# chhylp123/hifiasm

Measured on AMD Instinct MI355X. Metric: read-pair overlaps/sec (sum ol->length / (ha_pt_gen + all-reads h_ec_lchain pass)), higher is better.
Workload: dtype u64 hashing / int32 + f64 chain scores

## Files before the change

### hifiasm_amd/csrc/hao_capi.hip

```cpp
#include <algorithm>
#include <cmath>
#include <cstring>
#include "hao_ctx.hpp"
#include "hao_sketch.cuh"
#include "hao_select2.cuh"
#include "hao_host.hpp"
#include "hao_index.cuh"
#include "hao_query.cuh"
#include "hao_chain.cuh"
#include "hao_deliver.cuh"
#include "hao_comm.hpp"
#include "hao_gather.hpp"
#include "hao_pipeline.hpp"
#include "hao_tables.hpp"
#include "hao_batch.hpp"
#include "hao_files.hpp"

extern "C" {

void hao_opt_default(hao_opt_t *o)
{
	memset(o, 0, sizeof(*o));
	o->k = 51; o->w = 51; o->hpc = 1; o->sample_dist = 500; o->rewin = 1000; o->min_hist_cnt = 5;
	o->max_kmer_cnt = 2000; o->max_n_chain = 100; o->high_factor = 5.0; o->is_ont = 0; o->hg_size = -1;
}

int hao_create(int device, const hao_opt_t *opt, hao_ctx **out)
{
	*out = nullptr;
	int n = 0;
	if (hipGetDeviceCount(&n) != hipSuccess || n <= 0 || device >= n) return HAO_ENODEV;
	if (hipSetDevice(device) != hipSuccess) return HAO_ENODEV;
	if (!opt || opt->k <= 0 || opt->k > 63 || opt->w <= 0 || opt->w >= 256) return HAO_EINVAL;
	hao_ctx *c = new hao_ctx();
	c->device = device; c->opt = *opt; c->max_n_chain = opt->max_n_chain; c->sw.load();
	{ int ncu = 0; if (hipDeviceGetAttribute(&ncu, hipDeviceAttributeMultiprocessorCount, device) == hipSuccess && ncu > 0) c->n_cu = ncu; }
	{
		int lo_ = 0, hi_ = 0; (void)hipDeviceGetStreamPriorityRange(&lo_, &hi_);
		if (hipStreamCreateWithPriority(&c->stream, hipStreamDefault, lo_) != hipSuccess) { delete c; return HAO_ENODEV; }
	}
	if (hipHostMalloc((void**)&c->peek_h, HAO_PEEK_WORDS * 8, hipHostMallocMapped) != hipSuccess || hipHostGetDevicePointer((void**)&c->peek_d, c->peek_h, 0) != hipSuccess) { (void)hipStreamDestroy(c->stream); delete c; return HAO_ENOMEM; }
	memset(c->ft_hist, 0, sizeof(c->ft_hist)); memset(c->pt_hist, 0, sizeof(c->pt_hist));
	*out = c;
	return HAO_OK;
}

void hao_destroy(hao_ctx *c)
{
	if (!c) return;
	(void)hipSetDevice(c->device);
	(void)hipStreamSynchronize(c->stream);
	delete c->batch; c->batch = nullptr;
	if (c->comm) { if (c->comm->nccl) ncclCommDestroy(c->comm->nccl); delete c->comm; c->comm = nullptr; }
	const hipStream_t st = c->stream; unsigned long long *const peek_h = c->peek_h;
	delete c;
	(void)hipStreamDestroy(st);
	if (peek_h) (void)hipHostFree(peek_h);
}

const char *hao_last_error(const hao_ctx *c) { return c ? c->err.c_str() : "null ctx"; }

#define HAO_NOT_ON_VIEW(c, what) do { if ((c)->owner) { hao_set_err((c), what ": not on an attached batch context (hao_attach)"); return HAO_EINVAL; } } while (0)

int hao_attach(hao_ctx *o, hao_ctx **out)
{
	if (!o || !out) return HAO_EINVAL;
	*out = nullptr;
	if (o->owner) { hao_set_err(o, "hao_attach: attach to the owning engine, not to another view"); return HAO_EINVAL; }
	hao_ctx *c = nullptr;
	if (int rc = hao_create(o->device, &o->opt, &c)) return rc;
	c->owner = o; c->attached_gen = ~0ULL;
	*out = c;
	return HAO_OK;
}

int hao_set_reads(hao_ctx *c, const uint8_t *packed, const uint64_t *pk_off, const uint32_t *len, uint64_t n_reads,
				  const uint64_t *nsite_off, const uint32_t *nsite)
{
	if (!c || !packed || !pk_off || !len) return HAO_EINVAL;
	HAO_NOT_ON_VIEW(c, "hao_set_reads"); ++c->index_gen;
	hao_gather_drop(c);
	if (n_reads >= (1ULL << 28)) { hao_set_err(c, "more than 2^28 reads (htab.cpp:765)"); return HAO_EUNSUPP; }
	HIP_TRY(hipSetDevice(c->device));
	c->n_reads = n_reads; c->n_pk_bytes = pk_off[n_reads]; c->max_len = 0;
	c->h_len.assign(len, len + n_reads);
	c->n_bases = 0;
	for (uint64_t i = 0; i < n_reads; ++i) {
		if (len[i] >= (1u << 27)) { hao_set_err(c, "read longer than 2^27 (htab.h:13-18)"); return HAO_EUNSUPP; }
		c->n_bases += len[i];
	}
	HIP_TRY(c->d_packed.reserve(c->n_pk_bytes + 16)); HIP_TRY(c->d_pk_off.reserve(n_reads + 1)); HIP_TRY(c->d_len.reserve(n_reads + 1));
	HIP_TRY(hipMemcpyAsync(c->d_packed.p, packed, c->n_pk_bytes, hipMemcpyHostToDevice, c->stream));
	HIP_TRY(hipMemsetAsync(c->d_packed.p + c->n_pk_bytes, 0, 16, c->stream));
	HIP_TRY(hipMemcpyAsync(c->d_pk_off.p, pk_off, (n_reads + 1) * 8, hipMemcpyHostToDevice, c->stream));
	HIP_TRY(hipMemcpyAsync(c->d_len.p, len, n_reads * 4, hipMemcpyHostToDevice, c->stream));
	c->has_n = nsite_off && nsite && nsite_off[n_reads] > 0;
	c->h_nsite_off.clear();
	if (c->has_n) {
		c->h_nsite_off.assign(nsite_off, nsite_off + n_reads + 1);
		HIP_TRY(c->d_nsite_off.reserve(n_reads + 1)); HIP_TRY(c->d_nsite.reserve(nsite_off[n_reads] + 1));
		HIP_TRY(hipMemcpyAsync(c->d_nsite_off.p, nsite_off, (n_reads + 1) * 8, hipMemcpyHostToDevice, c->stream));
		HIP_TRY(hipMemcpyAsync(c->d_nsite.p, nsite, nsite_off[n_reads] * 4, hipMemcpyHostToDevice, c->stream));
	}
	c->rid_base = 0; c->n_total = n_reads; c->h_len_all = c->h_len;
	c->max_len_all = 0; for (uint64_t i = 0; i < n_reads; ++i) c->max_len_all = std::max(c->max_len_all, len[i]);
	HIP_TRY(c->d_len_all.reserve(n_reads + 1));
	HIP_TRY(hipMemcpyAsync(c->d_len_all.p, len, n_reads * 4, hipMemcpyHostToDevice, c->stream));
	HIP_TRY(hipStreamSynchronize(c->stream));
	c->has_ft = false; c->has_pt = false; c->h_ix_valid = false; c->sk_n = 0;
	return HAO_OK;
}

int hao_set_shard(hao_ctx *c, uint64_t rid_base, uint64_t n_total, const uint32_t *all_len)
{
	if (!c || !all_len || rid_base + c->n_reads > n_total) return HAO_EINVAL;
	HAO_NOT_ON_VIEW(c, "hao_set_shard"); ++c->index_gen;
	hao_gather_drop(c);
	if (n_total >= (1ULL << 28)) { hao_set_err(c, "more than 2^28 reads (htab.cpp:765)"); return HAO_EUNSUPP; }
	for (uint64_t i = 0; i < c->n_reads; ++i) if (all_len[rid_base + i] != c->h_len[i]) { hao_set_err(c, "all_len disagrees with the local read lengths"); return HAO_EINVAL; }
	HIP_TRY(hipSetDevice(c->device));
	c->rid_base = rid_base; c->n_total = n_total; c->h_len_all.assign(all_len, all_len + n_total); c->max_len = 0;
	c->max_len_all = 0; for (uint64_t i = 0; i < n_total; ++i) c->max_len_all = std::max(c->max_len_all, all_len[i]);
	HIP_TRY(c->d_len_all.reserve(n_total + 1));
	HIP_TRY(hipMemcpy(c->d_len_all.p, all_len, n_total * 4, hipMemcpyHostToDevice));
	c->has_ft = false; c->has_pt = false; c->h_ix_valid = false;
	return HAO_OK;
}

int hao_dist_unique_id(uint8_t id[128])
{
	ncclUniqueId u; if (ncclGetUniqueId(&u) != ncclSuccess) return HAO_ENODEV;
	static_assert(sizeof(ncclUniqueId) <= 128, "ncclUniqueId");
	memset(id, 0, 128); memcpy(id, &u, sizeof(u));
	return HAO_OK;
}

int hao_dist_init(hao_ctx *c, const uint8_t id[128], int rank, int world)
{
	if (!c || !id || rank < 0 || rank >= world) return HAO_EINVAL;
	HAO_NOT_ON_VIEW(c, "hao_dist_init");
	HIP_TRY(hipSetDevice(c->device));
	if (!c->comm) c->comm = new hao_comm();
	ncclUniqueId u; memcpy(&u, id, sizeof(u));
	c->comm->rank = rank; c->comm->world = world; c->comm->loop = nullptr;
	{
		int rt = 0; NCCL_TRY(ncclGetVersion(&rt));
		const int rt_major = rt >= 10000 ? rt / 10000 : rt / 1000;
		if (rt_major != NCCL_MAJOR) { hao_set_err(c, "RCCL major version " + std::to_string(rt_major) + " at run time, " + std::to_string(NCCL_MAJOR) + " at compile time"); return HAO_EUNSUPP; }
	}
	NCCL_TRY(ncclCommInitRank(&c->comm->nccl, world, u, rank));
	return HAO_OK;
}

void *hao_loop_create(int world)
{
	hao_loop_group *g = new hao_loop_group();
	g->world = world; pthread_barrier_init(&g->bar, nullptr, world); g->ptr.assign(world, nullptr); g->ptr2.assign(world, nullptr); g->cnt.resize(world); g->hostv.resize(world);
	return g;
}
void hao_loop_destroy(void *grp) { if (grp) { hao_loop_group *g = (hao_loop_group*)grp; pthread_barrier_destroy(&g->bar); delete g; } }
int hao_dist_init_loopback(hao_ctx *c, void *grp, int rank)
{
	if (!c || !grp) return HAO_EINVAL;
	hao_loop_group *g = (hao_loop_group*)grp;
	if (rank < 0 || rank >= g->world) return HAO_EINVAL;
	if (!c->comm) c->comm = new hao_comm();
	c->comm->rank = rank; c->comm->world = g->world; c->comm->loop = g; c->comm->nccl = nullptr;
	return HAO_OK;
}

int hao_sketch_batch(hao_ctx *c, uint64_t rid_lo, uint64_t rid_hi, int use_ft, int sample_dist)
{
	if (!c || rid_lo > rid_hi || rid_hi > c->n_reads) return HAO_EINVAL;
	HAO_NOT_ON_VIEW(c, "hao_sketch_batch");
	HIP_TRY(hipSetDevice(c->device));
	c->timer.begin(c->stream);
	int rc = hao_sketch_run(c, rid_lo, rid_hi, use_ft && c->has_ft, sample_dist, 1);
	if (rc != HAO_OK) return rc;
	HIP_TRY(hipStreamSynchronize(c->stream));
	c->timer.collect(c->stage_ms);
	c->h_mz_off.resize(c->sk_n + 1);
	HIP_TRY(hipMemcpy(c->h_mz_off.data(), c->d_mz_off.p, (c->sk_n + 1) * 8, hipMemcpyDeviceToHost));
	return HAO_OK;
}

int hao_fetch_sketch(hao_ctx *c, uint64_t rid, const hao_mz_t **mz, uint64_t *n)
{
	if (!c || rid < c->sk_lo || rid >= c->sk_lo + c->sk_n || c->h_mz_off.size() != c->sk_n + 1) return HAO_EINVAL;
	HIP_TRY(hipSetDevice(c->device));
	uint64_t s = c->h_mz_off[rid - c->sk_lo], e = c->h_mz_off[rid - c->sk_lo + 1], m = e - s;
	c->h_mz_fetch.resize(m + 1);
	std::vector<uint64_t> x(m + 1), info(m + 1);
	if (m) {
		HIP_TRY(hipMemcpy(x.data(), c->d_mz_x.p + s, m * 8, hipMemcpyDeviceToHost));
		HIP_TRY(hipMemcpy(info.data(), c->d_mz_info.p + s, m * 8, hipMemcpyDeviceToHost));
	}
	for (uint64_t i = 0; i < m; ++i) { c->h_mz_fetch[i].x = x[i]; c->h_mz_fetch[i].info = info[i]; }
	*mz = c->h_mz_fetch.data(); *n = m;
	return HAO_OK;
}

int hao_stage_times(hao_ctx *c, const char **names, float *ms, int cap)
{
	if (!c) return 0;
	int n = 0;
	for (auto &p : c->stage_ms) { if (n >= cap) break; names[n] = p.first.c_str(); ms[n] = p.second; ++n; }
	return n;
}

}

#include "hao_capi_rest.hpp"
#include "hao_sortdbg.hpp"
```

### hifiasm_amd/csrc/hao_ctx.hpp

```cpp
#pragma once
#include <time.h>
#include <rocprim/rocprim.hpp>
#include <map>
#include <algorithm>
#include <cstdlib>
#include <cstring>
#include <type_traits>
#include "hao_common.cuh"
#include "hao_grid_pair.cuh"

struct hao_ctx;
static void hao_set_err(hao_ctx *c, const std::string &m);

template<typename T> struct DevBuf {
	T *p = nullptr; size_t cap = 0; bool borrowed = false;
	DevBuf() = default;
	DevBuf(const DevBuf&) = delete; DevBuf &operator=(const DevBuf&) = delete;
	DevBuf(DevBuf &&o) noexcept : p(o.p), cap(o.cap), borrowed(o.borrowed) { o.p = nullptr; o.cap = 0; o.borrowed = false; }
	DevBuf &operator=(DevBuf &&o) noexcept { if (this != &o) { release(); p = o.p; cap = o.cap; borrowed = o.borrowed; o.p = nullptr; o.cap = 0; o.borrowed = false; } return *this; }
	~DevBuf() { release(); }
	hipError_t reserve(size_t n) {
		if (n <= cap) return hipSuccess;
		if (borrowed) return hipErrorInvalidValue;
		if (p) (void)hipFree(p);
		p = nullptr; cap = 0;
		size_t want = n + n / 8 + 64;
		hipError_t e = hipMalloc((void**)&p, want * sizeof(T));
		if (e == hipSuccess) cap = want;
		return e;
	}
	hipError_t reserve_exact(size_t n) {
		if (n <= cap) return hipSuccess;
		if (borrowed) return hipErrorInvalidValue;
		if (p) (void)hipFree(p);
		p = nullptr; cap = 0;
		hipError_t e = hipMalloc((void**)&p, n * sizeof(T));
		if (e == hipSuccess) cap = n;
		return e;
	}
	void release() { if (p && !borrowed) (void)hipFree(p); p = nullptr; cap = 0; borrowed = false; }
	void borrow(const DevBuf<T> &o) { release(); p = o.p; cap = o.cap; borrowed = o.p != nullptr; }
};

inline bool hao_dbg_sync = false;
struct StageTimer {
	std::vector<std::string> names; std::vector<hipEvent_t> ev; std::vector<double> host_t; hipStream_t st = nullptr;
	static double now() { struct timespec ts; clock_gettime(CLOCK_MONOTONIC, &ts); return ts.tv_sec + 1e-9 * ts.tv_nsec; }
	void begin(hipStream_t s) { st = s; names.clear(); host_t.clear(); mark("__begin"); }
	void mark(const char *name) {
		size_t i = names.size();
		if (i >= ev.size()) { hipEvent_t e; (void)hipEventCreate(&e); ev.push_back(e); }
		names.push_back(name); host_t.push_back(now()); (void)hipEventRecord(ev[i], st);
		if (hao_dbg_sync) { const hipError_t e = hipStreamSynchronize(st); fprintf(stderr, "[stage] %s: %s\n", name, hipGetErrorString(e)); fflush(stderr); }
	}
	void collect(std::vector<std::pair<std::string, float> > &out) {
		out.clear();
		for (size_t i = 1; i < names.size(); ++i) { float ms = 0; (void)hipEventElapsedTime(&ms, ev[i - 1], ev[i]); out.push_back(std::make_pair(names[i], ms)); }
		for (size_t i = 1; i < names.size(); ++i) if (names[i].compare(0, 3, "ft_") == 0) out.push_back(std::make_pair("host_" + names[i], (float)((host_t[i] - host_t[i - 1]) * 1e3)));
	}
	~StageTimer() { for (auto e : ev) (void)hipEventDestroy(e); }
};

struct hao_switches {
	bool seedphase = false, qcphase = false, dp_stats = false, selphase = false, dltime = false, bloom = false;
	bool seq_chain = false, dp_seqtail = false, dp_nospec = false, dp_serial = false, seq_prune = false, seed_noql = false, al_coop = false;
	long long sk_gcap = -1, exc_cap = -1, ft_chunk_slots = 0; unsigned long long gather_chunk = 64ULL << 20, al_slice = 4ULL << 30, ix_pad = 0, sort40_min = 1ULL << 23; int fc_raw_every = 0, exc_every = 0; bool qmz_raw = false, arena_probe = false;
	int arena_numa = 3, seed_merge_maxn = 24000, seed_lds_ratio = 120, ft_passes = 0, seed_lds = 1;
	static bool in_list(const char *v, const char *name) {
		const size_t n = strlen(name);
		for (const char *p = v; p && *p; ) { const char *e = strchr(p, ','); const size_t l = e ? (size_t)(e - p) : strlen(p); if (l == n && strncmp(p, name, n) == 0) return true; p = e ? e + 1 : nullptr; }
		return false;
	}
	static bool in_kv(const char *v, const char *name, unsigned long long &out) {
		const size_t n = strlen(name);
		for (const char *p = v; p && *p; ) { const char *e = strchr(p, ','); if (strncmp(p, name, n) == 0 && p[n] == '=') { out = strtoull(p + n + 1, nullptr, 10); return true; } p = e ? e + 1 : nullptr; }
		return false;
	}
	void load() {
		if (const char *v = getenv("HAO_DBG_PRINT")) {
			seedphase = in_list(v, "seed"); qcphase = in_list(v, "qc"); dp_stats = in_list(v, "dp"); selphase = in_list(v, "sel"); dltime = in_list(v, "dl"); bloom = in_list(v, "bloom"); hao_dbg_sync = in_list(v, "sync");
		}
		if (const char *v = getenv("HAO_DBG_FORCE")) {
			seq_chain = in_list(v, "seq_chain");
			dp_seqtail = in_list(v, "dp_seqtail");
			dp_nospec = in_list(v, "dp_nospec");
			dp_serial = in_list(v, "dp_serial");
			seq_prune = in_list(v, "seq_prune");
			seed_noql = in_list(v, "noql");
			al_coop = in_list(v, "al_coop");
		}
		if (const char *v = getenv("HAO_DBG_TEST")) {
			unsigned long long x;
			if (in_kv(v, "ix_pad", x)) ix_pad = x;
			if (in_kv(v, "sort40_min", x)) sort40_min = x;
			if (in_kv(v, "sk_gcap", x)) sk_gcap = (long long)x;
			if (in_kv(v, "exc_cap", x)) exc_cap = (long long)x;
			if (in_kv(v, "fc_raw_every", x)) fc_raw_every = (int)x;
			if (in_kv(v, "exc_every", x)) exc_every = (int)x;
			if (in_kv(v, "qmz_raw", x)) qmz_raw = x != 0;
			if (in_kv(v, "arena_probe", x)) arena_probe = x != 0;
			if (in_kv(v, "ft_chunk_slots", x)) ft_chunk_slots = (long long)x;
			if (in_kv(v, "al_slice", x)) al_slice = std::max<unsigned long long>(x, 8);
			if (in_kv(v, "gather_chunk", x)) gather_chunk = std::max<unsigned long long>(x, 64);
		}
		if (const char *e = getenv("HAO_SEED_LDS")) seed_lds = atoi(e) ? 1 : 0;
		if (const char *e = getenv("HAO_SEED_LDS_RATIO")) seed_lds_ratio = std::max(0, atoi(e));
		if (const char *e = getenv("HAO_SEED_MERGE_MAXN")) seed_merge_maxn = std::max(0, atoi(e));
		if (const char *e = getenv("HAO_FT_PASSES")) ft_passes = std::max(0, atoi(e));
		if (const char *e = getenv("HAO_ARENA_NUMA")) arena_numa = atoi(e);
	}
};

static __global__ void hao_peek_kernel(const unsigned long long *src, int n, unsigned long long *dst)
{ if ((int)threadIdx.x < n) dst[threadIdx.x] = src[threadIdx.x]; }
enum hao_peek_id : int {
	PK_ANCHORS, PK_CLS_BASE,
	PK_N_CHAINS, PK_N_CL, PK_N_FC_RAW, PK_N_OL, PK_N_FC,
	PK_N_EXC, PK_N_CODES, PK_N_FCW, PK_SEED_OVF, PK_ERR, PK_SLOW,
	PK_GRID_PAIRS, PK_REF_SLOTS, PK_REF_UNRES,
	PK_SORT40,
	PK_TG_TRACED, PK_TG_CTR, PK_TG_NCIG,
	PK_RS_SIZES, PK_RS_WAITING, PK_RS_TOTAL, PK_RS_NWINS,
	PK_WL_N, PK_WL_PLAN, PK_WL_NCIG, PK_WL_CTR,
	PK_LD_SETUP, PK_LD_ROUND, PK_LD_SEL, PK_LD_END,
	PK_COUNT
};
struct hao_peek_rng { int at, n; };
static constexpr hao_peek_rng HAO_PEEK[PK_COUNT] = {
	 {0, 1},  {1, 8},
	 {9, 1},  {10, 1},  {11, 1},  {12, 1},  {13, 1},
	 {14, 1},  {15, 1},  {19, 1},  {20, 3},  {23, 1},  {64, 11},
	 {32, 1},  {37, 1},  {38, 1},
	 {16, 3},
	 {33, 1},  {34, 2},  {36, 1},
	 {40, 2},  {42, 1},  {43, 1},  {44, 1},
	 {48, 1},  {49, 3},  {52, 1},  {53, 6},
	 {80, 2},  {82, 48},  {130, 16},  {146, 2},
};
constexpr int HAO_PEEK_WORDS = 512;
constexpr bool hao_peek_table_ok()
{
	for (int i = 0; i < PK_COUNT; ++i) {
		if (HAO_PEEK[i].at < 0 || HAO_PEEK[i].n < 1 || HAO_PEEK[i].at + HAO_PEEK[i].n > HAO_PEEK_WORDS) return false;
		for (int j = 0; j < i; ++j) if (HAO_PEEK[i].at < HAO_PEEK[j].at + HAO_PEEK[j].n && HAO_PEEK[j].at < HAO_PEEK[i].at + HAO_PEEK[i].n) return false;
	}
	return true;
}
static_assert(hao_peek_table_ok(), "read-back slots: a range beyond the mapped words, or two ranges that overlap");

struct WinResident {
	enum Stage { NONE, ED, RESCUE, WLIST };
	void on_new_batch() { *this = WinResident(); }
	void on_host_fed() { owner = NOBODY; n = 0; trace = false; }
	void on_grid(uint64_t pairs) { owner = GRID; n = pairs; lists = false; }
	void on_ref_begin(Stage s) { if (chain >= s) chain = (Stage)(s - 1); host &= (1u << s) - 1; if (s == ED) { owner = NOBODY; n = 0; } lists = false; }
	void on_ref_done(Stage s, uint64_t pairs = 0) { chain = s; if (s == ED) { owner = REF; n = pairs; } if (s == WLIST) lists = true; }
	void on_host_copy(Stage s) { host |= 1u << s; }
	void on_trace_grid(bool done) { trace = done; }
	uint64_t scratch_pairs() const { return owner == NOBODY ? 0 : n; }
	bool ed_resident() const { return chain >= ED; } bool rescue_resident() const { return chain >= RESCUE; } bool trace_resident() const { return trace; }
	bool ref_input_resident() const { return chain >= ED && owner == REF; }
	bool wlist_input_resident() const { return chain >= RESCUE && owner == REF; }
	bool wlist_resident() const { return chain >= WLIST && owner == REF; }
	bool wlist_records_resident() const { return lists; }
	bool host_current(Stage s) const { return (host >> s) & 1u; }
private:
	enum Owner { NOBODY, GRID, REF } owner = NOBODY; uint64_t n = 0; Stage chain = NONE; uint32_t host = 0; bool trace = false, lists = false;
};

struct hao_ref_io {
	const hao_ovlp_t *ol; uint64_t n_ol;
	uint32_t wl; const uint8_t *tab;
	const hao_ed_pair *pairs; uint64_t n_pairs, n_slots;
	const hao_ed_result_t *res; const uint8_t *err8; const uint16_t *pe16;
	DevBuf<hao_rs_ovlp> *rs_ovlp; DevBuf<uint64_t> *rs_off; DevBuf<hao_rs_win> *rs_wins;
	DevBuf<uint64_t> *wl_woff; DevBuf<hao_rs_win> *wl_wins; DevBuf<uint64_t> *wl_cigoff; DevBuf<uint16_t> *wl_cig;
};

struct hao_ctx {
	int device = 0; hao_opt_t opt; std::string err; hipStream_t stream = nullptr; hao_switches sw;
	hao_ctx *owner = nullptr; uint64_t index_gen = 0, attached_gen = 0;
	unsigned long long *peek_h = nullptr, *peek_d = nullptr;
	unsigned long long peeked(hao_peek_id slot, int k = 0) const { return peek_h[HAO_PEEK[slot].at + k]; }
	uint64_t n_reads = 0, n_bases = 0, n_pk_bytes = 0; bool has_n = false; uint32_t max_len = 0;
	DevBuf<uint8_t> d_packed; DevBuf<uint64_t> d_pk_off; DevBuf<uint32_t> d_len; DevBuf<uint64_t> d_nsite_off; DevBuf<uint32_t> d_nsite;
	std::vector<uint32_t> h_len; std::vector<uint64_t> h_nsite_off;
	uint64_t rid_base = 0, n_total = 0; uint32_t max_len_all = 0; int n_cu = 256; DevBuf<uint32_t> d_len_all; std::vector<uint32_t> h_len_all; struct hao_comm *comm = nullptr;
	bool gs_valid = false, gs_has_n = false; uint64_t gs_pk_bytes = 0, gs_nsites = 0;
	DevBuf<uint8_t> g_packed; DevBuf<uint64_t> g_pk_off, g_nsite_off; DevBuf<uint32_t> g_nsite;
	bool has_ft = false; int ft_peak_hom = -1, ft_peak_het = -1, ft_cutoff = 0, ft_passes_used = 1; int64_t ft_hist[HAO_N_COUNTS];
	std::vector<uint64_t> h_ft_keys; std::vector<int32_t> h_ft_vals;
	DevBuf<uint64_t> d_ft_keys; DevBuf<int32_t> d_ft_vals; DevBuf<uint32_t> d_ft_bucket;
	DevBuf<uint32_t> d_ft_hbit; DevBuf<unsigned long long> d_ft_hslot; int ft_hbits = 0;
	int max_n_chain = 100, hom_cov = -1, het_cov = -1;
	uint64_t sk_lo = 0, sk_n = 0, sk_total = 0; bool sk_is_index = false;
	DevBuf<uint64_t> d_tile_off; DevBuf<uint32_t> d_tile_ord, d_n_runs, d_tot_l; DevBuf<uint64_t> d_chunk_off, d_chunk_cnt64;
	DevBuf<uint8_t> d_scalar_flag; DevBuf<uint32_t> d_scalar_list, d_unit_rid;
	DevBuf<uint64_t> d_pool_x, d_pool_info; DevBuf<uint32_t> d_pool_ord; DevBuf<unsigned long long> d_cursor; DevBuf<int> d_err;
	DevBuf<uint64_t> d_chunk_base, d_chunk_dst; DevBuf<uint32_t> d_chunk_cnt;
	DevBuf<uint64_t> d_g_x, d_g_info; DevBuf<uint32_t> d_g_ord; DevBuf<uint64_t> d_g_off; DevBuf<uint32_t> d_new_n; DevBuf<uint64_t> d_new_n64;
	DevBuf<uint64_t> d_mz_x, d_mz_info, d_mz_off;
	DevBuf<unsigned char> d_tmp; DevBuf<unsigned char> d_ring; DevBuf<uint32_t> d_ringord, d_cnt_ws;
	std::vector<uint64_t> h_mz_off; std::vector<hao_mz_t> h_mz_fetch;
	bool has_pt = false; int64_t pt_hist[HAO_N_COUNTS];
	uint64_t ix_n_mz = 0, ix_n_sorted = 0, ix_n_keys = 0, ix_n_pos = 0, ix_pad = 0; int ix_bucket_bits = 16;
	DevBuf<uint64_t> d_ix_mz_x, d_ix_mz_info, d_ix_mz_off;
	DevBuf<uint64_t> d_ix_sx, d_ix_sinfo;
	DevBuf<uint64_t> d_ix_lk; bool lk_valid = false; DevBuf<uint32_t> w_runid;
	DevBuf<uint64_t> d_ix_keys, d_ix_start; DevBuf<uint32_t> d_ix_cnt; DevBuf<uint32_t> d_ix_bucket;
	DevBuf<uint64_t> w_ukeys, w_flag, w_kpos, w_ustart; DevBuf<uint32_t> w_ucnt; DevBuf<unsigned long long> w_hist; DevBuf<uint32_t> w_ok, w_ok2, w_oi, w_oi2;
	DevBuf<uint32_t> w_s40_list, w_s40_o; DevBuf<uint64_t> w_s40_x, w_lkv2; DevBuf<unsigned long long> w_s40_cnt; uint64_t s40_runs = 0;
	std::vector<uint64_t> h_ix_keys, h_ix_off, h_ix_pos, h_ix_mz_off; bool h_ix_valid = false;
	WinResident win;
	DevBuf<hao_ed_task_t> al_task; DevBuf<uint64_t> al_k1, al_k2, al_path; DevBuf<uint32_t> al_i1, al_order, al_sel; DevBuf<hao_ed_result_t> al_res; DevBuf<hao_trace_result_t> al_tres;
	DevBuf<uint8_t> al_want; DevBuf<uint16_t> al_cig;
	uint32_t ded_window = 0, ded_thre = 0;
	uint32_t ded_place = 0; double ded_erate = 0; DevBuf<uint8_t> ded_tab;
	struct RefGrid {
		DevBuf<uint64_t> cnt, woff; DevBuf<int16_t> shift; DevBuf<uint8_t> werr; DevBuf<hao_ed_pair> pairs; DevBuf<unsigned long long> ctr;
	} rf;
	DevBuf<uint8_t> rf_tab; uint32_t rf_tab_wl = 0; double rf_tab_erate = 0; DevBuf<hao_ed_ovlp_sum> rf_sum; std::vector<hao_ed_ovlp_sum> rf_hsum; uint64_t rf_unres = 0, rs_wc = 0;
	struct Rescue {
		DevBuf<uint16_t> wpe; DevBuf<uint64_t> rbase, path, off; DevBuf<hao_rs_state> st; DevBuf<hao_rs_win> rec, wins; DevBuf<hao_rs_ovlp> ovlp; DevBuf<unsigned long long> ctr;
		std::vector<hao_rs_ovlp> h_ovlp; std::vector<uint64_t> h_win_off; std::vector<hao_rs_win> h_wins;
	} rs;
	uint64_t rs_slots = 0, rs_rounds = 0, rs_active = 0, rs_total = 0, rs_nw = 0;
	struct Wlist {
		DevBuf<uint64_t> cnt, woff, ncig, cig_off, key, key2, path; DevBuf<hao_wl_plan> plan; DevBuf<hao_rs_win> wins; DevBuf<uint32_t> idx, sel, rowof; DevBuf<uint16_t> rows, cig; DevBuf<unsigned long long> ctr;
		std::vector<uint64_t> h_woff, h_cig_off, r_woff, r_cig_off; std::vector<hao_rs_win> h_wins; std::vector<uint16_t> h_cig;
	} wl;
	uint64_t wl_out[5] = { 0, 0, 0, 0, 0 };
	struct Ladder {
		DevBuf<hao_ladder_req_t> req; DevBuf<hao_ladder_res_t> res; DevBuf<int32_t> att; DevBuf<uint64_t> ncig, rowref, off, poff, selcnt; DevBuf<uint32_t> open[2], sel; DevBuf<hao_ld_coord> coord;
		DevBuf<uint16_t> rows[5], cig; DevBuf<unsigned long long> ctr;
		DevBuf<hao_ladder_adv_res_t> res_adv; DevBuf<uint32_t> xlist; DevBuf<uint16_t> xrow; DevBuf<int32_t> pth;
		DevBuf<int64_t> est;
		DevBuf<hao_ladder_req_t> e_req; DevBuf<int64_t> e_est; DevBuf<unsigned long long> e_ctr;
	} ld;
	uint64_t ld_n = 0;
	bool ld_valid = false, ld_adv = false; uint64_t ld_ncig = 0, ld_rounds[5] = { 0, 0, 0, 0, 0 };
	struct TraceGrid {
		DevBuf<uint8_t> want; DevBuf<uint32_t> sel; DevBuf<uint64_t> cnt, loc, off, path; DevBuf<uint16_t> rows; DevBuf<unsigned long long> ctr;
	} tg;
	uint32_t tg_wl = 0, tg_thre = 0; uint64_t tg_n = 0, tg_nsel = 0, tg_ncig = 0, tg_nuntr = 0;
	DevBuf<hao_ed_pair> tg_pairs; DevBuf<uint8_t> tg_err; DevBuf<uint16_t> tg_pe, tg_ps, tg_ncig16, tg_cig;
	struct Batch;
	Batch *batch = nullptr;
	StageTimer timer; std::vector<std::pair<std::string, float> > stage_ms;
};

static void hao_set_err(hao_ctx *c, const std::string &m) { if (c) c->err = m; }

#define HAO_CHECK_LAUNCH() HIP_TRY(hipGetLastError())

static int hao_peek(hao_ctx *c, const void *src, int words, hao_peek_id slot)
{
	if (words > HAO_PEEK[slot].n) { hao_set_err(c, "hao_peek: more words than the slot holds"); return HAO_EINVAL; }
	hipLaunchKernelGGL(hao_peek_kernel, dim3(1), dim3(64), 0, c->stream, (const unsigned long long*)src, words, c->peek_d + HAO_PEEK[slot].at); HAO_CHECK_LAUNCH();
	return HAO_OK;
}

static bool hao_comm_is_active(const struct hao_comm *cm);
static inline bool hao_is_sharded(const hao_ctx *c) { const hao_ctx *o = c->owner ? c->owner : c; return o->comm && hao_comm_is_active(o->comm); }

struct hao_read_view {
	const uint8_t *packed; const uint64_t *pk_off; const uint32_t *len; const uint64_t *nsite_off; const uint32_t *nsite;
	const uint32_t *h_len; uint64_t n, id_base, local0;
};
static inline bool hao_reads_view(const hao_ctx *c, hao_read_view *V)
{
	if (!hao_is_sharded(c)) {
		V->packed = c->d_packed.p; V->pk_off = c->d_pk_off.p; V->len = c->d_len.p; V->nsite_off = c->has_n ? c->d_nsite_off.p : nullptr; V->nsite = c->has_n ? c->d_nsite.p : nullptr;
		V->h_len = c->h_len.data(); V->n = c->n_reads; V->id_base = c->rid_base; V->local0 = 0;
		return true;
	}
	if (!c->gs_valid) return false;
	V->packed = c->g_packed.p; V->pk_off = c->g_pk_off.p; V->len = c->d_len_all.p; V->nsite_off = c->gs_has_n ? c->g_nsite_off.p : nullptr; V->nsite = c->gs_has_n ? c->g_nsite.p : nullptr;
	V->h_len = c->h_len_all.data(); V->n = c->n_total; V->id_base = 0; V->local0 = c->rid_base;
	return true;
}
#define HAO_STAGE_VIEW(c, V, what) hao_read_view V; do { if (!hao_reads_view((c), &V)) { hao_set_err((c), what ": single-device mode only"); return HAO_EUNSUPP; } } while (0)

static inline hipError_t hao_tmp(hao_ctx *c, size_t bytes) { return c->d_tmp.reserve(bytes + 256); }

template<typename F>
static int hao_rocprim(hao_ctx *c, F run)
{
	size_t tb = 0;
	HIP_TRY(run((void*)nullptr, tb));
	HIP_TRY(hao_tmp(c, tb));
	HIP_TRY(run((void*)c->d_tmp.p, tb));
	return HAO_OK;
}
template<typename In, typename Out>
static int hao_excl_scan_u64(hao_ctx *c, In in, Out out, size_t n)
{
	return hao_rocprim(c, [&](void *tmp, size_t &tb) { return rocprim::exclusive_scan(tmp, tb, in, out, (uint64_t)0, n, rocprim::plus<uint64_t>(), c->stream); });
}
template<typename K, typename V>
static int hao_sort_pairs(hao_ctx *c, K *k_in, K *k_out, V *v_in, V *v_out, size_t n, unsigned bits)
{
	return hao_rocprim(c, [&](void *tmp, size_t &tb) { return rocprim::radix_sort_pairs(tmp, tb, k_in, k_out, v_in, v_out, n, 0, bits, c->stream); });
}
template<typename In, typename F, typename Out>
static int hao_select(hao_ctx *c, In in, F flags_or_pred, Out out, uint64_t *count, size_t n)
{
	return hao_rocprim(c, [&](void *tmp, size_t &tb) {
		if constexpr (std::is_pointer<F>::value) return rocprim::select(tmp, tb, in, flags_or_pred, out, count, n, c->stream);
		else return rocprim::select(tmp, tb, in, out, count, n, flags_or_pred, c->stream);
	});
}

static inline uint64_t hao_col_slice(const hao_ctx *c, uint64_t n, uint64_t bytes_per_pair)
{
	return std::max<uint64_t>(256, std::min<uint64_t>((n + 255) & ~255ULL, (c->sw.al_slice / bytes_per_pair) & ~255ULL));
}
#define HAO_SCRATCH_KEEP (1ULL << 30)
template<typename T> static inline void hao_release_above(DevBuf<T> &b, uint64_t bytes) { if ((uint64_t)b.cap * sizeof(T) > bytes) b.release(); }

static int hao_view_refresh(hao_ctx *c)
{
	hao_ctx *o = c->owner;
	if (!o || c->attached_gen == o->index_gen) return HAO_OK;
	c->opt = o->opt;
	c->n_reads = o->n_reads; c->n_bases = o->n_bases; c->n_pk_bytes = o->n_pk_bytes; c->has_n = o->has_n; c->max_len = o->max_len;
	c->rid_base = o->rid_base; c->n_total = o->n_total; c->max_len_all = o->max_len_all; c->n_cu = o->n_cu; c->max_n_chain = o->max_n_chain; c->hom_cov = o->hom_cov; c->het_cov = o->het_cov;
	c->has_pt = o->has_pt; c->ix_n_mz = o->ix_n_mz; c->ix_n_sorted = o->ix_n_sorted; c->ix_n_keys = o->ix_n_keys; c->ix_n_pos = o->ix_n_pos; c->ix_pad = o->ix_pad; c->ix_bucket_bits = o->ix_bucket_bits; c->lk_valid = o->lk_valid;
	c->h_len = o->h_len; c->h_nsite_off = o->h_nsite_off; c->h_len_all = o->h_len_all; c->h_ix_mz_off = o->h_ix_mz_off;
	c->d_packed.borrow(o->d_packed); c->d_pk_off.borrow(o->d_pk_off); c->d_len.borrow(o->d_len); c->d_len_all.borrow(o->d_len_all); c->d_nsite_off.borrow(o->d_nsite_off); c->d_nsite.borrow(o->d_nsite);
	c->gs_valid = o->gs_valid; c->gs_has_n = o->gs_has_n; c->gs_pk_bytes = o->gs_pk_bytes; c->gs_nsites = o->gs_nsites;
	c->g_packed.borrow(o->g_packed); c->g_pk_off.borrow(o->g_pk_off); c->g_nsite_off.borrow(o->g_nsite_off); c->g_nsite.borrow(o->g_nsite);
	c->d_ix_mz_x.borrow(o->d_ix_mz_x); c->d_ix_mz_info.borrow(o->d_ix_mz_info); c->d_ix_mz_off.borrow(o->d_ix_mz_off); c->d_ix_sinfo.borrow(o->d_ix_sinfo); c->d_ix_lk.borrow(o->d_ix_lk);
	c->d_ix_keys.borrow(o->d_ix_keys); c->d_ix_start.borrow(o->d_ix_start); c->d_ix_cnt.borrow(o->d_ix_cnt); c->d_ix_bucket.borrow(o->d_ix_bucket);
	c->attached_gen = o->index_gen;
	return HAO_OK;
}
```

### hifiasm_amd/csrc/hao_gather.hpp

```cpp
#pragma once
#include "hao_ctx.hpp"
#include "hao_comm.hpp"
#include "hao_deliver.cuh"

__global__ void hao_gather_rebase_kernel(const uint64_t *tab, int W, uint64_t n_total, uint64_t *pk_off, uint64_t *nsite_off)
{
	const uint64_t i = (uint64_t)blockIdx.x * blockDim.x + threadIdx.x;
	if (i > n_total) return;
	const uint64_t *start = tab, *pkb = tab + (W + 1), *nsb = tab + 2 * (W + 1), *hn = tab + 3 * (W + 1);
	if (i == n_total) { pk_off[i] = pkb[W]; if (nsite_off) nsite_off[i] = nsb[W]; return; }
	int lo = 0, hi = W;
	while (hi - lo > 1) { const int mid = (lo + hi) >> 1; if (start[mid] <= i) lo = mid; else hi = mid; }
	pk_off[i] += pkb[lo];
	if (nsite_off) nsite_off[i] = hn[lo] ? nsite_off[i] + nsb[lo] : nsb[lo];
}

__global__ __launch_bounds__(256) void hao_reads_digest_kernel(hao_read_view V, unsigned long long *out)
{
	const uint64_t r = (uint64_t)blockIdx.x * 4 + (threadIdx.x >> 6); const uint32_t lane = threadIdx.x & 63;
	__shared__ uint64_t part[2][4];
	uint64_t b = 0, s = 0;
	if (r < V.n) {
		const uint32_t L = V.len[r]; const uint64_t nb = (uint64_t)L / 4 + 1, nw = (nb + 7) / 8;
		const uintptr_t a = (uintptr_t)(V.packed + V.pk_off[r]); const uint64_t *W = (const uint64_t*)(a & ~(uintptr_t)7); const uint32_t sh = (uint32_t)(a & 7) * 8;
		for (uint64_t j = lane; j < nw; j += 64) {
			uint64_t w = W[j] >> sh; if (sh) w |= W[j + 1] << (64 - sh);
			const uint64_t rem = nb - 8 * j; if (rem < 8) w &= (1ULL << (8 * rem)) - 1;
			b += hao_dg_term(5, j + 1, w);
		}
		uint64_t m = 0;
		if (V.nsite_off) {
			const uint64_t s0 = V.nsite_off[r]; m = V.nsite_off[r + 1] - s0;
			for (uint64_t k = lane; k < m; k += 64) s += hao_dg_term(6, k + 1, V.nsite[s0 + k]);
		}
#pragma unroll
		for (int dl = 32; dl >= 1; dl >>= 1) { b += __shfl_xor(b, dl); s += __shfl_xor(s, dl); }
		b = hao_dg_term(7, r, b + hao_dg_term(5, 0, L)); s = hao_dg_term(8, r, s + hao_dg_term(6, 0, m));
	}
	if (lane == 0) { part[0][threadIdx.x >> 6] = b; part[1][threadIdx.x >> 6] = s; }
	__syncthreads();
	if (threadIdx.x == 0) {
		atomicAdd(out, (unsigned long long)(part[0][0] + part[0][1] + part[0][2] + part[0][3]));
		atomicAdd(out + 1, (unsigned long long)(part[1][0] + part[1][1] + part[1][2] + part[1][3]));
	}
}

static void hao_gather_drop(hao_ctx *c)
{ c->gs_valid = false; c->gs_has_n = false; c->gs_pk_bytes = c->gs_nsites = 0; c->g_packed.release(); c->g_pk_off.release(); c->g_nsite_off.release(); c->g_nsite.release(); }

static int hao_gather_bytes(hao_ctx *c, hao_comm &cm, const void *src, const std::vector<uint64_t> &cnt, const std::vector<uint64_t> &at, void *dst, uint64_t chunk, DevBuf<char> &stage)
{
	const int W = cm.world; uint64_t maxc = 0;
	for (int r = 0; r < W; ++r) maxc = std::max(maxc, cnt[r]);
	std::vector<uint64_t> part(W);
	for (uint64_t off = 0; off < maxc; off += chunk) {
		for (int r = 0; r < W; ++r) part[r] = cnt[r] > off ? std::min(chunk, cnt[r] - off) : 0;
		if (int rc = hao_comm_allgatherv(c, cm, (const char*)src + (part[cm.rank] ? off : 0), part[cm.rank], 1, stage.p, part)) return rc;
		uint64_t d = 0;
		for (int r = 0; r < W; ++r) if (part[r]) { HIP_TRY(hipMemcpyAsync((char*)dst + at[r] + off, stage.p + d, part[r], hipMemcpyDeviceToDevice, c->stream)); d += part[r]; }
	}
	return HAO_OK;
}

static int hao_gather_reads_run(hao_ctx *c)
{
	hao_comm &cm = *c->comm; const int W = cm.world;
	const uint64_t mine[4] = { c->n_reads, c->rid_base, c->n_pk_bytes, c->has_n ? c->h_nsite_off[c->n_reads] : 0 };
	std::vector<uint64_t> all;
	if (int rc = hao_comm_allgather_u64n(c, cm, mine, 4, all)) return rc;
	std::vector<uint64_t> tab(4 * (size_t)W + 3, 0), c_pk(W), c_off(W), c_nso(W), c_ns(W), a_pk(W), a_off(W), a_ns(W);
	uint64_t *start = tab.data(), *pkb = start + W + 1, *nsb = pkb + W + 1, *hn = nsb + W + 1;
	int local_rc = HAO_OK;
	for (int r = 0; r < W; ++r) {
		const uint64_t *v = &all[4 * (size_t)r];
		if (v[1] != start[r]) { hao_set_err(c, "hao_dist_gather_reads: the shards are not contiguous slices of the reads in rank order (rank " + std::to_string(r) + ")"); local_rc = HAO_EINVAL; }
		start[r + 1] = start[r] + v[0]; pkb[r + 1] = pkb[r] + v[2]; nsb[r + 1] = nsb[r] + v[3]; hn[r] = v[3] != 0;
		c_pk[r] = v[2]; c_off[r] = v[0] * 8; c_nso[r] = v[3] ? v[0] * 8 : 0; c_ns[r] = v[3] * 4;
		a_pk[r] = pkb[r]; a_off[r] = start[r] * 8; a_ns[r] = nsb[r] * 4;
	}
	if (!local_rc && start[W] != c->n_total) { hao_set_err(c, "hao_dist_gather_reads: the shards hold " + std::to_string(start[W]) + " reads, hao_set_shard announced " + std::to_string(c->n_total)); local_rc = HAO_EINVAL; }
	const uint64_t n = c->n_total, PK = pkb[W], NS = nsb[W], chunk = c->sw.gather_chunk;
	uint64_t share = 0; for (int r = 0; r < W; ++r) share = std::max(share, std::max(std::max(c_pk[r], c_off[r]), c_ns[r]));
	DevBuf<char> stage; DevBuf<uint64_t> d_tab;
	auto alloc = [&]() -> int {
		HIP_TRY(c->g_packed.reserve_exact(PK + 16)); HIP_TRY(c->g_pk_off.reserve_exact(n + 1));
		if (NS) { HIP_TRY(c->g_nsite_off.reserve_exact(n + 1)); HIP_TRY(c->g_nsite.reserve_exact(NS + 1)); }
		HIP_TRY(stage.reserve_exact(std::min(chunk, share) * (uint64_t)W + 16)); HIP_TRY(d_tab.reserve_exact(tab.size()));
		HIP_TRY(hipMemsetAsync(c->g_packed.p + PK, 0, 16, c->stream));
		HIP_TRY(hipMemcpyAsync(d_tab.p, tab.data(), tab.size() * 8, hipMemcpyHostToDevice, c->stream));
		return HAO_OK;
	};
	if (!local_rc) local_rc = alloc();
	{ std::vector<uint64_t> st; if (int rc = hao_comm_allgather_u64(c, cm, 0, st, local_rc)) return rc; }
	if (int rc = hao_gather_bytes(c, cm, c->d_packed.p, c_pk, a_pk, c->g_packed.p, chunk, stage)) return rc;
	if (int rc = hao_gather_bytes(c, cm, c->d_pk_off.p, c_off, a_off, c->g_pk_off.p, chunk, stage)) return rc;
	if (NS) {
		if (int rc = hao_gather_bytes(c, cm, c->d_nsite_off.p, c_nso, a_off, c->g_nsite_off.p, chunk, stage)) return rc;
		if (int rc = hao_gather_bytes(c, cm, c->d_nsite.p, c_ns, a_ns, c->g_nsite.p, chunk, stage)) return rc;
	}
	hipLaunchKernelGGL(hao_gather_rebase_kernel, dim3((unsigned)((n + 256) / 256)), dim3(256), 0, c->stream, (const uint64_t*)d_tab.p, W, n, c->g_pk_off.p, NS ? c->g_nsite_off.p : nullptr);
	local_rc = hipGetLastError() == hipSuccess && hipStreamSynchronize(c->stream) == hipSuccess ? HAO_OK : HAO_ENODEV;
	if (local_rc) hao_set_err(c, "hao_dist_gather_reads: the offsets' kernel failed");
	{ std::vector<uint64_t> st; if (int rc = hao_comm_allgather_u64(c, cm, 0, st, local_rc)) return rc; }
	c->gs_valid = true; c->gs_has_n = NS != 0; c->gs_pk_bytes = PK; c->gs_nsites = NS;
	return HAO_OK;
}

extern "C" {

int hao_dist_gather_reads(hao_ctx *c)
{
	if (!c) return HAO_EINVAL;
	if (c->owner) { hao_set_err(c, "hao_dist_gather_reads: not on an attached batch context (hao_attach)"); return HAO_EINVAL; }
	if (!hao_is_sharded(c) || c->gs_valid) return HAO_OK;
	HIP_TRY(hipSetDevice(c->device));
	++c->index_gen;
	const int rc = hao_gather_reads_run(c);
	if (rc) hao_gather_drop(c);
	return rc;
}

int hao_reads_digest(hao_ctx *c, uint64_t out[2])
{
	if (!c || !out) return HAO_EINVAL;
	if (int rc = hao_view_refresh(c)) return rc;
	HAO_STAGE_VIEW(c, V, "hao_reads_digest needs the bases of all reads");
	HIP_TRY(hipSetDevice(c->device));
	HIP_TRY(c->d_cursor.reserve(2));
	HIP_TRY(hipMemsetAsync(c->d_cursor.p, 0, 16, c->stream));
	if (V.n) { hipLaunchKernelGGL(hao_reads_digest_kernel, dim3((unsigned)((V.n + 3) / 4)), dim3(256), 0, c->stream, V, c->d_cursor.p); HAO_CHECK_LAUNCH(); }
	HIP_TRY(hipMemcpyAsync(out, c->d_cursor.p, 16, hipMemcpyDeviceToHost, c->stream));
	HIP_TRY(hipStreamSynchronize(c->stream));
	return HAO_OK;
}

}
```

### hifiasm_amd/csrc/hao_pipeline.hpp

```cpp
#pragma once
#include "hao_ctx.hpp"
#include "hao_sketch.cuh"
#include "hao_sketch3.cuh"

struct U32ToU64 { __host__ __device__ uint64_t operator()(uint32_t v) const { return v; } };

__global__ void hao_chunk_count_kernel(const uint32_t *n_runs, const uint8_t *scalar_flag, uint64_t n_sel, int k, int chunk, uint64_t *cnt)
{
	uint64_t r = (uint64_t)blockIdx.x * blockDim.x + threadIdx.x;
	if (r > n_sel) return;
	if (r == n_sel) { cnt[r] = 0; return; }
	uint64_t nm = n_runs[r] >= (uint32_t)k ? n_runs[r] - k + 1 : 0;
	cnt[r] = scalar_flag[r] ? 1 : (nm == 0 ? 1 : (nm + chunk - 1) / chunk);
}

__global__ void hao_unit_rid_kernel(const uint64_t *chunk_off, uint64_t n_sel, uint32_t *unit_rid)
{
	const uint64_t r = (uint64_t)blockIdx.x * blockDim.x + threadIdx.x;
	if (r >= n_sel) return;
	for (uint64_t u = chunk_off[r]; u < chunk_off[r + 1]; ++u) unit_rid[u] = (uint32_t)r;
}

static hao_ft_dev hao_ft_view(hao_ctx *c)
{
	hao_ft_dev f; f.keys = c->d_ft_keys.p; f.vals = c->d_ft_vals.p; f.bucket = c->d_ft_bucket.p; f.n = c->h_ft_keys.size();
	f.hbit = c->d_ft_hbit.p; f.hslot = (const ulonglong2*)c->d_ft_hslot.p; f.hbits = c->ft_hbits;
	return f;
}

static int hao_sketch_run(hao_ctx *c, uint64_t lo, uint64_t hi, int use_ft, int sample_dist, int stamp_rid)
{
	const uint64_t n_sel = hi - lo; const int k = c->opt.k, w = c->opt.w;
	const bool unit_variant = w == 51 && k == 51;
	const bool wave_variant = w == 51 && k + 7 <= 64;
	const int chunk = unit_variant ? hao_sk3<51, 51>::MW : (wave_variant ? hao_sk2<51>::CHUNK : HAO_SK_CHUNK);
	c->sk_lo = lo; c->sk_n = n_sel; c->sk_total = 0;
	HIP_TRY(c->d_mz_off.reserve(n_sel + 2));
	if (n_sel == 0) { HIP_TRY(hipMemsetAsync(c->d_mz_off.p, 0, 8, c->stream)); return HAO_OK; }
	std::vector<uint64_t> tile_off(n_sel + 1); std::vector<uint8_t> flag(n_sel); std::vector<uint32_t> slist; uint64_t nb = 0;
	const bool even_k = (k & 1) == 0;
	for (uint64_t r = 0; r < n_sel; ++r) {
		uint32_t L = c->h_len[lo + r];
		tile_off[r] = r == 0 ? 0 : tile_off[r - 1] + (c->h_len[lo + r - 1] + HAO_SK_TILE - 1) / HAO_SK_TILE + 1;
		bool hasn = c->has_n && c->h_nsite_off[lo + r + 1] > c->h_nsite_off[lo + r];
		flag[r] = (hasn || even_k) ? 1 : 0;
		if (flag[r]) slist.push_back((uint32_t)r);
		nb += L;
	}
	tile_off[n_sel] = tile_off[n_sel - 1] + (c->h_len[hi - 1] + HAO_SK_TILE - 1) / HAO_SK_TILE + 1;
	HIP_TRY(c->d_tile_off.reserve(n_sel + 1)); HIP_TRY(c->d_tile_ord.reserve(tile_off[n_sel] + 1)); HIP_TRY(c->d_n_runs.reserve(n_sel + 1));
	HIP_TRY(c->d_tot_l.reserve(n_sel + 1)); HIP_TRY(c->d_scalar_flag.reserve(n_sel + 1)); HIP_TRY(c->d_scalar_list.reserve(slist.size() + 1));
	HIP_TRY(c->d_chunk_off.reserve(n_sel + 2)); HIP_TRY(c->d_chunk_cnt64.reserve(n_sel + 2)); HIP_TRY(c->d_cursor.reserve(2)); HIP_TRY(c->d_err.reserve(2));
	HIP_TRY(hipMemcpyAsync(c->d_tile_off.p, tile_off.data(), (n_sel + 1) * 8, hipMemcpyHostToDevice, c->stream));
	HIP_TRY(hipMemcpyAsync(c->d_scalar_flag.p, flag.data(), n_sel, hipMemcpyHostToDevice, c->stream));
	if (!slist.empty()) HIP_TRY(hipMemcpyAsync(c->d_scalar_list.p, slist.data(), slist.size() * 4, hipMemcpyHostToDevice, c->stream));
	c->timer.mark("sk_h2d");
	hipLaunchKernelGGL(hpc_index_kernel, dim3((unsigned)((n_sel + 3) / 4)), dim3(256), 0, c->stream, c->d_packed.p, c->d_pk_off.p, c->d_len.p,
					   c->d_tile_off.p, c->d_tile_ord.p, c->d_n_runs.p, lo, n_sel, c->opt.hpc, unit_variant ? c->d_scalar_flag.p : (uint8_t*)nullptr);
	HAO_CHECK_LAUNCH();
	hipLaunchKernelGGL(hao_chunk_count_kernel, dim3((unsigned)((n_sel + 256) / 256)), dim3(256), 0, c->stream, c->d_n_runs.p, c->d_scalar_flag.p, n_sel, k, chunk, c->d_chunk_cnt64.p);
	HAO_CHECK_LAUNCH();
	if (int rc = hao_excl_scan_u64(c, c->d_chunk_cnt64.p, c->d_chunk_off.p, n_sel + 1)) return rc;
	HIP_TRY(hipMemcpyAsync(c->d_tot_l.p, c->d_n_runs.p, n_sel * 4, hipMemcpyDeviceToDevice, c->stream));
	uint64_t n_chunks = 0;
	HIP_TRY(hipMemcpyAsync(&n_chunks, c->d_chunk_off.p + n_sel, 8, hipMemcpyDeviceToHost, c->stream));
	if (unit_variant) HIP_TRY(hipMemcpyAsync(flag.data(), c->d_scalar_flag.p, n_sel, hipMemcpyDeviceToHost, c->stream));
	HIP_TRY(hipStreamSynchronize(c->stream));
	if (unit_variant) {
		const size_t n0 = slist.size(); slist.clear();
		for (uint64_t r = 0; r < n_sel; ++r) if (flag[r]) slist.push_back((uint32_t)r);
		if (slist.size() != n0) { HIP_TRY(c->d_scalar_list.reserve(slist.size() + 1)); HIP_TRY(hipMemcpyAsync(c->d_scalar_list.p, slist.data(), slist.size() * 4, hipMemcpyHostToDevice, c->stream)); }
	}
	c->timer.mark("sk_index");
	HIP_TRY(c->d_chunk_base.reserve(n_chunks + 1)); HIP_TRY(c->d_chunk_cnt.reserve(n_chunks + 1)); HIP_TRY(c->d_chunk_dst.reserve(n_chunks + 2));
	if (unit_variant) {
		HIP_TRY(c->d_unit_rid.reserve(n_chunks + 1));
		hipLaunchKernelGGL(hao_unit_rid_kernel, dim3((unsigned)((n_sel + 255) / 256)), dim3(256), 0, c->stream, c->d_chunk_off.p, n_sel, c->d_unit_rid.p);
		HAO_CHECK_LAUNCH();
	}
	if (!slist.empty()) { HIP_TRY(c->d_ring.reserve(slist.size() * 256 * sizeof(hao_cand))); HIP_TRY(c->d_ringord.reserve(slist.size() * 256)); HIP_TRY(c->d_cnt_ws.reserve(slist.size() + 1)); }
	const size_t smem = hao_sk_smem_bytes(w, k);
	const uint64_t pool_static = unit_variant ? n_chunks * SK3_SLOT : 0;
	uint64_t cap = pool_static + nb / (unit_variant ? 32 : 6) + 65536, gcap = std::min(nb / 6 + 65536, nb / 16 + 65536), total = 0;
	if (c->sw.sk_gcap >= 0) gcap = (uint64_t)c->sw.sk_gcap;
	hao_scalar_args sa;
	for (int attempt = 0; ; ++attempt) {
		HIP_TRY(c->d_pool_x.reserve(cap)); HIP_TRY(c->d_pool_info.reserve(cap)); HIP_TRY(c->d_pool_ord.reserve(cap));
		HIP_TRY(hipMemsetAsync(c->d_cursor.p, 0, 8, c->stream)); HIP_TRY(hipMemsetAsync(c->d_err.p, 0, 4, c->stream));
		HIP_TRY(hipMemsetAsync(c->d_chunk_cnt.p, 0, (n_chunks + 1) * 4, c->stream));
		if (!slist.empty()) {
			sa.packed = c->d_packed.p; sa.pk_off = c->d_pk_off.p; sa.len = c->d_len.p; sa.nsite_off = c->has_n ? c->d_nsite_off.p : nullptr; sa.nsite = c->has_n ? c->d_nsite.p : nullptr;
			sa.chunk_off = c->d_chunk_off.p; sa.scalar_flag = c->d_scalar_flag.p; sa.scalar_list = c->d_scalar_list.p; sa.n_scalar = (uint32_t)slist.size();
			sa.rid_lo = lo; sa.k = k; sa.w = w; sa.hpc = c->opt.hpc; sa.use_ft = use_ft; sa.ft = hao_ft_view(c);
			sa.ring_ws = (hao_cand*)c->d_ring.p; sa.ringord_ws = c->d_ringord.p;
			sa.pool_x = c->d_pool_x.p; sa.pool_info = c->d_pool_info.p; sa.pool_ord = c->d_pool_ord.p; sa.pool_cursor = c->d_cursor.p; sa.pool_cap = cap;
			sa.chunk_base = c->d_chunk_base.p; sa.chunk_cnt = c->d_chunk_cnt.p; sa.tot_l = c->d_tot_l.p; sa.err = c->d_err.p; sa.pass = 0; sa.cnt_ws = c->d_cnt_ws.p; sa.pool_static = pool_static;
			hipLaunchKernelGGL(sketch_scalar_kernel, dim3((unsigned)((slist.size() + 63) / 64)), dim3(64), 0, c->stream, sa);
			HAO_CHECK_LAUNCH();
		}
		hao_sk_args a;
		a.packed = c->d_packed.p; a.pk_off = c->d_pk_off.p; a.len = c->d_len.p; a.tile_off = c->d_tile_off.p; a.tile_ord = c->d_tile_ord.p; a.n_runs = c->d_n_runs.p;
		a.chunk_off = c->d_chunk_off.p; a.scalar_flag = c->d_scalar_flag.p; a.rid_lo = lo; a.n_sel = n_sel; a.k = k; a.w = w; a.hpc = c->opt.hpc; a.ft = hao_ft_view(c);
		a.pool_x = c->d_pool_x.p; a.pool_info = c->d_pool_info.p; a.pool_ord = c->d_pool_ord.p; a.pool_cursor = c->d_cursor.p; a.pool_cap = cap;
		a.chunk_base = c->d_chunk_base.p; a.chunk_cnt = c->d_chunk_cnt.p; a.err = c->d_err.p; a.pool_static = pool_static; a.unit_rid = c->d_unit_rid.p; a.n_units = n_chunks;
		if (unit_variant) {
			if (use_ft && a.ft.n > 0) hipLaunchKernelGGL((sketch_unit_kernel<true, 51, 51>), dim3((unsigned)((n_chunks + 3) / 4)), dim3(256), 0, c->stream, a);
			else hipLaunchKernelGGL((sketch_unit_kernel<false, 51, 51>), dim3((unsigned)((n_chunks + 3) / 4)), dim3(256), 0, c->stream, a);
		} else if (wave_variant) {
			if (use_ft && a.ft.n > 0) hipLaunchKernelGGL((sketch_chunk_wave_kernel<true, 51>), dim3((unsigned)n_chunks), dim3(256), 0, c->stream, a);
			else hipLaunchKernelGGL((sketch_chunk_wave_kernel<false, 51>), dim3((unsigned)n_chunks), dim3(256), 0, c->stream, a);
		} else if (use_ft && a.ft.n > 0) hipLaunchKernelGGL(sketch_chunk_kernel<true>, dim3((unsigned)n_chunks), dim3(HAO_SK_THREADS), smem, c->stream, a);
		else hipLaunchKernelGGL(sketch_chunk_kernel<false>, dim3((unsigned)n_chunks), dim3(HAO_SK_THREADS), smem, c->stream, a);
		HAO_CHECK_LAUNCH();
		c->timer.mark("sk_chunks");
		{
			auto it = rocprim::make_transform_iterator(c->d_chunk_cnt.p, U32ToU64());
			if (int rc = hao_excl_scan_u64(c, it, c->d_chunk_dst.p, n_chunks + 1)) return rc;
		}
		if (!slist.empty()) { sa.pass = 1; hipLaunchKernelGGL(sketch_scalar_kernel, dim3((unsigned)((slist.size() + 63) / 64)), dim3(64), 0, c->stream, sa); HAO_CHECK_LAUNCH(); }
		const bool thin = use_ft && a.ft.n > 0 && sample_dist > w;
		HIP_TRY(c->d_g_off.reserve(n_sel + 2)); HIP_TRY(c->d_mz_x.reserve(gcap + 1)); HIP_TRY(c->d_mz_info.reserve(gcap + 1));
		hipLaunchKernelGGL(sketch_read_off_kernel, dim3((unsigned)((n_sel + 256) / 256)), dim3(256), 0, c->stream, c->d_chunk_off.p, c->d_chunk_dst.p, n_sel, c->d_g_off.p);
		HAO_CHECK_LAUNCH();
		if (!thin) {
			HIP_TRY(hipMemcpyAsync(c->d_mz_off.p, c->d_g_off.p, (n_sel + 1) * 8, hipMemcpyDeviceToDevice, c->stream));
			hipLaunchKernelGGL(sketch_gather_finish_kernel, dim3((unsigned)((n_sel + 3) / 4)), dim3(256), 0, c->stream, c->d_pool_x.p, c->d_pool_info.p, c->d_chunk_base.p, c->d_chunk_cnt.p,
							   c->d_chunk_dst.p, c->d_chunk_off.p, lo + c->rid_base, n_sel, stamp_rid, c->d_mz_x.p, c->d_mz_info.p, gcap, c->d_err.p);
			HAO_CHECK_LAUNCH();
			c->timer.mark("sk_gather");
		} else {
			HIP_TRY(c->d_g_x.reserve(gcap + 1)); HIP_TRY(c->d_g_info.reserve(gcap + 1)); HIP_TRY(c->d_g_ord.reserve(gcap + 1));
			hipLaunchKernelGGL(sketch_gather_kernel, dim3((unsigned)((n_chunks + 3) / 4)), dim3(256), 0, c->stream, c->d_pool_x.p, c->d_pool_info.p, c->d_pool_ord.p,
							   c->d_chunk_base.p, c->d_chunk_cnt.p, c->d_chunk_dst.p, n_chunks, c->d_g_x.p, c->d_g_info.p, c->d_g_ord.p, gcap, c->d_err.p);
			HAO_CHECK_LAUNCH();
			c->timer.mark("sk_gather");
			HIP_TRY(c->d_new_n.reserve(n_sel + 2)); HIP_TRY(hipMemsetAsync(c->d_new_n.p + n_sel, 0, 4, c->stream));
			{
				hipLaunchKernelGGL((sketch_select2_kernel<HAO_S2_CAP_SMALL, 64>), dim3((unsigned)n_sel), dim3(64), 0, c->stream, c->d_g_x.p, c->d_g_info.p, c->d_g_ord.p, c->d_g_off.p,
								   c->d_len.p, c->d_tot_l.p, lo, n_sel, sample_dist, c->opt.rewin, k, c->d_new_n.p, c->d_err.p);
				HAO_CHECK_LAUNCH();
				hipLaunchKernelGGL((sketch_select2_kernel<HAO_S2_CAP, 256>), dim3((unsigned)n_sel), dim3(256), 0, c->stream, c->d_g_x.p, c->d_g_info.p, c->d_g_ord.p, c->d_g_off.p,
								   c->d_len.p, c->d_tot_l.p, lo, n_sel, sample_dist, c->opt.rewin, k, c->d_new_n.p, c->d_err.p);
			}
			HAO_CHECK_LAUNCH();
			auto it = rocprim::make_transform_iterator(c->d_new_n.p, U32ToU64());
			if (int rc = hao_excl_scan_u64(c, it, c->d_mz_off.p, n_sel + 1)) return rc;
			c->timer.mark("sk_select");
			hipLaunchKernelGGL(sketch_finish_kernel, dim3((unsigned)((n_sel + 3) / 4)), dim3(256), 0, c->stream, c->d_g_x.p, c->d_g_info.p, c->d_g_off.p, c->d_mz_off.p, lo + c->rid_base, n_sel, stamp_rid,
							   c->d_mz_x.p, c->d_mz_info.p, c->d_err.p);
			HAO_CHECK_LAUNCH();
		}
		int err = 0;
		HIP_TRY(hipMemcpyAsync(&err, c->d_err.p, 4, hipMemcpyDeviceToHost, c->stream));
		HIP_TRY(hipMemcpyAsync(&total, c->d_mz_off.p + n_sel, 8, hipMemcpyDeviceToHost, c->stream));
		HIP_TRY(hipStreamSynchronize(c->stream));
		if (!err) break;
		if (attempt >= 3) { hao_set_err(c, "minimizer pool overflow"); return HAO_ENOMEM; }
		cap = pool_static + (attempt == 0 ? nb / 2 + 65536 : nb + 65536); gcap = cap - pool_static;
	}
	c->sk_total = total;
	c->timer.mark("sk_finish");
	return HAO_OK;
}
```

### hifiasm_amd/csrc/hao_tables.hpp

```cpp
#pragma once
#include <chrono>
#include "hao_comm.hpp"
#include "hao_pipeline.hpp"
#include "hao_index.cuh"
#include "hao_host.hpp"

__global__ void hao_lower_bound_kernel(const uint64_t *keys, uint64_t n, const uint64_t *targets, int nt, uint64_t *out)
{
	int t = blockIdx.x * blockDim.x + threadIdx.x;
	if (t >= nt) return;
	uint64_t lo = 0, hi = n, x = targets[t];
	while (lo < hi) { uint64_t m = (lo + hi) >> 1; if (keys[m] < x) lo = m + 1; else hi = m; }
	out[t] = lo;
}
__global__ void hao_lower_bound_low12_kernel(const uint64_t *keys, uint64_t n, const uint64_t *targets, int nt, uint64_t *out)
{
	int t = blockIdx.x * blockDim.x + threadIdx.x;
	if (t >= nt) return;
	uint64_t lo = 0, hi = n, x = targets[t];
	while (lo < hi) { uint64_t m = (lo + hi) >> 1; if ((keys[m] & 4095) < x) lo = m + 1; else hi = m; }
	out[t] = lo;
}
__global__ void hao_owner_key_kernel(const uint64_t *x, uint64_t n, uint32_t *key, uint32_t *idx)
{
	uint64_t i = (uint64_t)blockIdx.x * blockDim.x + threadIdx.x;
	if (i < n) { key[i] = (uint32_t)(x[i] >> 48); idx[i] = (uint32_t)i; }
}
__global__ void hao_gather2_kernel(const uint32_t *idx, const uint64_t *a, const uint64_t *b, uint64_t n, uint64_t *oa, uint64_t *ob)
{
	uint64_t i = (uint64_t)blockIdx.x * blockDim.x + threadIdx.x;
	if (i < n) { const uint32_t j = idx[i]; oa[i] = a[j]; ob[i] = b[j]; }
}
__global__ void hao_add_const_kernel(uint64_t *v, uint64_t n, uint64_t add)
{
	uint64_t i = (uint64_t)blockIdx.x * blockDim.x + threadIdx.x;
	if (i < n) v[i] += add;
}
__global__ void hao_add_u32_kernel(uint32_t *v, uint64_t n, uint32_t add)
{
	uint64_t i = (uint64_t)blockIdx.x * blockDim.x + threadIdx.x;
	if (i < n) v[i] += add;
}
__global__ void hao_adjdiff_kernel(const uint64_t *off, uint64_t n, uint64_t *cnt)
{
	uint64_t i = (uint64_t)blockIdx.x * blockDim.x + threadIdx.x;
	if (i < n) cnt[i] = off[i + 1] - off[i];
}

static int hao_prepare_runs(hao_ctx *c, uint64_t lo, uint64_t hi, bool force_scalar_all, std::vector<uint32_t> &slist)
{
	const uint64_t n_sel = hi - lo;
	std::vector<uint64_t> tile_off(n_sel + 1); std::vector<uint8_t> flag(n_sel);
	slist.clear();
	for (uint64_t r = 0; r < n_sel; ++r) {
		tile_off[r] = r == 0 ? 0 : tile_off[r - 1] + (c->h_len[lo + r - 1] + HAO_SK_TILE - 1) / HAO_SK_TILE + 1;
		bool hasn = c->has_n && c->h_nsite_off[lo + r + 1] > c->h_nsite_off[lo + r];
		flag[r] = (hasn || force_scalar_all) ? 1 : 0;
		if (flag[r]) slist.push_back((uint32_t)r);
	}
	tile_off[n_sel] = tile_off[n_sel - 1] + (c->h_len[hi - 1] + HAO_SK_TILE - 1) / HAO_SK_TILE + 1;
	HIP_TRY(c->d_tile_off.reserve(n_sel + 1)); HIP_TRY(c->d_tile_ord.reserve(tile_off[n_sel] + 1)); HIP_TRY(c->d_n_runs.reserve(n_sel + 1));
	HIP_TRY(c->d_scalar_flag.reserve(n_sel + 1)); HIP_TRY(c->d_scalar_list.reserve(slist.size() + 1));
	HIP_TRY(hipMemcpyAsync(c->d_tile_off.p, tile_off.data(), (n_sel + 1) * 8, hipMemcpyHostToDevice, c->stream));
	HIP_TRY(hipMemcpyAsync(c->d_scalar_flag.p, flag.data(), n_sel, hipMemcpyHostToDevice, c->stream));
	if (!slist.empty()) HIP_TRY(hipMemcpyAsync(c->d_scalar_list.p, slist.data(), slist.size() * 4, hipMemcpyHostToDevice, c->stream));
	hipLaunchKernelGGL(hpc_index_kernel, dim3((unsigned)((n_sel + 3) / 4)), dim3(256), 0, c->stream, c->d_packed.p, c->d_pk_off.p, c->d_len.p,
					   c->d_tile_off.p, c->d_tile_ord.p, c->d_n_runs.p, lo, n_sel, c->opt.hpc, (uint8_t*)nullptr);
	HAO_CHECK_LAUNCH();
	HIP_TRY(hipStreamSynchronize(c->stream));
	return HAO_OK;
}

static int hao_prior_hom(const hao_ctx *c)
{
	if (c->opt.hg_size <= 0) return -1;
	uint64_t bs = 0; for (uint32_t l : c->h_len_all) bs += l;
	return (int)(bs / (uint64_t)c->opt.hg_size);
}

static int hao_shard_layout_check(hao_ctx *c, hao_comm &cm, int local_rc)
{
	const uint64_t mine[3] = { c->n_reads, c->rid_base, c->n_total }; std::vector<uint64_t> all;
	if (int rc = hao_comm_allgather_u64n(c, cm, mine, 3, all, local_rc)) return rc;
	uint64_t b = 0; bool ok = true;
	for (int r = 0; r < cm.world; ++r) { ok = ok && all[3 * r + 1] == b && all[3 * r + 2] == all[2]; b += all[3 * r]; }
	if (!ok || b != all[2]) { hao_set_err(c, "shards are not contiguous read ranges in rank order"); return HAO_EINVAL; }
	return HAO_OK;
}
static int hao_comm_agree(hao_ctx *c, hao_comm &cm, int local_rc) { std::vector<uint64_t> t; return hao_comm_allgather_u64(c, cm, 0, t, local_rc); }

struct NotSentinel { __host__ __device__ bool operator()(const uint64_t &h) const { return h != UINT64_MAX; } };
struct RunHead { const uint64_t *k; __host__ __device__ uint64_t operator()(uint64_t i) const { return (i == 0 || k[i] != k[i - 1]) ? 1 : 0; } };
struct RunHead32 { const uint64_t *k; __host__ __device__ uint32_t operator()(uint64_t i) const { return (i == 0 || k[i] != k[i - 1]) ? 1u : 0u; } };

template<typename Key>
static int hao_rle(hao_ctx *c, const Key *sorted, uint64_t n, Key *ukeys, uint32_t *ucnt, uint64_t *d_n_runs)
{
	size_t tb = 0;
	if (n <= 0xffffffffULL) {
		HIP_TRY(rocprim::run_length_encode(nullptr, tb, sorted, (unsigned int)n, ukeys, ucnt, d_n_runs, c->stream)); HIP_TRY(hao_tmp(c, tb));
		HIP_TRY(rocprim::run_length_encode(c->d_tmp.p, tb, sorted, (unsigned int)n, ukeys, ucnt, d_n_runs, c->stream));
	} else {
		auto ones = rocprim::make_constant_iterator<uint32_t>(1);
		HIP_TRY(rocprim::reduce_by_key(nullptr, tb, sorted, ones, (size_t)n, ukeys, ucnt, d_n_runs, rocprim::plus<uint32_t>(), rocprim::equal_to<Key>(), c->stream)); HIP_TRY(hao_tmp(c, tb));
		HIP_TRY(rocprim::reduce_by_key(c->d_tmp.p, tb, sorted, ones, (size_t)n, ukeys, ucnt, d_n_runs, rocprim::plus<uint32_t>(), rocprim::equal_to<Key>(), c->stream));
	}
	return HAO_OK;
}
static int hao_memset_big(hao_ctx *c, void *p, int v, uint64_t bytes)
{
	for (uint64_t o = 0; o < bytes; o += 1ULL << 30) HIP_TRY(hipMemsetAsync((char*)p + o, v, (size_t)std::min<uint64_t>(1ULL << 30, bytes - o), c->stream));
	return HAO_OK;
}

struct hao_rle_out { uint64_t n_unique; };
static int hao_sort_rle_hist(hao_ctx *c, uint64_t *d_keys, uint64_t *d_keys_alt, uint64_t n, DevBuf<uint64_t> &ukeys, DevBuf<uint32_t> &ucnt, uint64_t *n_unique, int64_t hist[HAO_N_COUNTS], uint64_t **sorted_out, uint32_t bias = 0)
{
	*n_unique = 0; memset(hist, 0, sizeof(int64_t) * HAO_N_COUNTS); *sorted_out = d_keys;
	if (n == 0) return HAO_OK;
	size_t tb = 0;
	rocprim::double_buffer<uint64_t> db(d_keys, d_keys_alt);
	HIP_TRY(rocprim::radix_sort_keys(nullptr, tb, db, n, 0, 64, c->stream));
	HIP_TRY(hao_tmp(c, tb));
	HIP_TRY(rocprim::radix_sort_keys(c->d_tmp.p, tb, db, n, 0, 64, c->stream));
	uint64_t *sorted = db.current(); *sorted_out = sorted;
	HIP_TRY(c->d_cursor.reserve(2));
	uint64_t n_runs = 0;
	{
		auto heads = rocprim::make_transform_iterator(rocprim::make_counting_iterator<uint64_t>(0), RunHead{sorted});
		tb = 0;
		HIP_TRY(rocprim::reduce(nullptr, tb, heads, (uint64_t*)c->d_cursor.p, (uint64_t)0, n, rocprim::plus<uint64_t>(), c->stream));
		HIP_TRY(hao_tmp(c, tb));
		HIP_TRY(rocprim::reduce(c->d_tmp.p, tb, heads, (uint64_t*)c->d_cursor.p, (uint64_t)0, n, rocprim::plus<uint64_t>(), c->stream));
		HIP_TRY(hipMemcpyAsync(&n_runs, c->d_cursor.p, 8, hipMemcpyDeviceToHost, c->stream));
		HIP_TRY(hipStreamSynchronize(c->stream));
	}
	HIP_TRY(ukeys.reserve(n_runs + 1)); HIP_TRY(ucnt.reserve(n_runs + 1));
	if (int rc = hao_rle(c, sorted, n, ukeys.p, ucnt.p, (uint64_t*)c->d_cursor.p)) return rc;
	HIP_TRY(hipMemcpyAsync(n_unique, c->d_cursor.p, 8, hipMemcpyDeviceToHost, c->stream));
	HIP_TRY(hipStreamSynchronize(c->stream));
	if (bias && *n_unique) { hipLaunchKernelGGL(hao_add_u32_kernel, dim3((unsigned)((*n_unique + 255) / 256)), dim3(256), 0, c->stream, ucnt.p, *n_unique, bias); HAO_CHECK_LAUNCH(); }
	DevBuf<unsigned long long> dh; HIP_TRY(dh.reserve(HAO_N_COUNTS));
	HIP_TRY(hipMemsetAsync(dh.p, 0, HAO_N_COUNTS * 8, c->stream));
	unsigned nb = (unsigned)std::min<uint64_t>((*n_unique + 255) / 256, 2048);
	if (nb) hipLaunchKernelGGL(hao_count_hist_kernel, dim3(nb), dim3(256), 0, c->stream, ucnt.p, *n_unique, dh.p);
	HAO_CHECK_LAUNCH();
	HIP_TRY(hipMemcpyAsync(hist, dh.p, HAO_N_COUNTS * 8, hipMemcpyDeviceToHost, c->stream));
	HIP_TRY(hipStreamSynchronize(c->stream));
	return HAO_OK;
}

static int hao_keep_runs(hao_ctx *c, const uint64_t *ukeys, const uint32_t *ucnt, uint64_t n_unique, int lo, int hi,
						 DevBuf<uint64_t> &keys, DevBuf<uint64_t> *start, DevBuf<uint32_t> &cnt, uint64_t *n_kept, uint64_t *n_pos)
{
	*n_kept = 0; if (n_pos) *n_pos = 0;
	if (n_unique == 0) return HAO_OK;
	DevBuf<uint64_t> &flag = c->w_flag, &kpos = c->w_kpos, &ustart = c->w_ustart;
	HIP_TRY(flag.reserve(n_unique + 1)); HIP_TRY(kpos.reserve(n_unique + 1)); HIP_TRY(ustart.reserve(n_unique + 1));
	hipLaunchKernelGGL(hao_range_flag_kernel, dim3((unsigned)((n_unique + 256) / 256)), dim3(256), 0, c->stream, ucnt, n_unique, lo, hi, flag.p);
	HAO_CHECK_LAUNCH();
	if (int rc = hao_excl_scan_u64(c, flag.p, kpos.p, n_unique + 1)) return rc;
	{ auto it = rocprim::make_transform_iterator(ucnt, U32ToU64()); if (int rc = hao_excl_scan_u64(c, it, ustart.p, n_unique)) return rc; }
	HIP_TRY(hipMemcpyAsync(n_kept, kpos.p + n_unique, 8, hipMemcpyDeviceToHost, c->stream));
	HIP_TRY(hipStreamSynchronize(c->stream));
	HIP_TRY(keys.reserve(*n_kept + 1)); HIP_TRY(cnt.reserve(*n_kept + 1)); if (start) HIP_TRY(start->reserve(*n_kept + 1));
	hipLaunchKernelGGL(hao_keep_scatter_kernel, dim3((unsigned)((n_unique + 255) / 256)), dim3(256), 0, c->stream, ukeys, ucnt, ustart.p, flag.p, kpos.p, n_unique,
					   keys.p, start ? start->p : nullptr, cnt.p);
	HAO_CHECK_LAUNCH();
	if (n_pos && *n_kept) {
		size_t tb = 0; auto it = rocprim::make_transform_iterator(cnt.p, U32ToU64());
		HIP_TRY(rocprim::reduce(nullptr, tb, it, (uint64_t*)c->d_cursor.p, (uint64_t)0, *n_kept, rocprim::plus<uint64_t>(), c->stream));
		HIP_TRY(hao_tmp(c, tb));
		HIP_TRY(rocprim::reduce(c->d_tmp.p, tb, it, (uint64_t*)c->d_cursor.p, (uint64_t)0, *n_kept, rocprim::plus<uint64_t>(), c->stream));
		HIP_TRY(hipMemcpyAsync(n_pos, c->d_cursor.p, 8, hipMemcpyDeviceToHost, c->stream));
	}
	HIP_TRY(hipStreamSynchronize(c->stream));
	return HAO_OK;
}

static int hao_build_bucket(hao_ctx *c, const uint64_t *keys, uint64_t n, int bits, DevBuf<uint32_t> &bucket)
{
	uint32_t nb = 1u << bits;
	HIP_TRY(bucket.reserve(nb + 2));
	hipLaunchKernelGGL(hao_bucket_kernel, dim3((nb + 256) / 256), dim3(256), 0, c->stream, keys, n, 64 - bits, nb, bucket.p);
	HAO_CHECK_LAUNCH();
	return HAO_OK;
}

static int hao_ft_build_hash(hao_ctx *c, uint64_t n)
{
	int hb = 15; while (hb < 32 && (1ULL << (hb - 2)) * 3 < n * 4) ++hb;
	c->ft_hbits = hb;
	const uint64_t nbk = 1ULL << (hb - 2), nw = (1ULL << hb) / 32;
	HIP_TRY(c->d_ft_hbit.reserve(nw + 1)); HIP_TRY(c->d_ft_hslot.reserve(2 * nbk + 2));
	HIP_TRY(hipMemsetAsync(c->d_ft_hbit.p, 0, nw * 4, c->stream));
	for (uint64_t o = 0; o < 2 * nbk * 8; o += 1ULL << 30) HIP_TRY(hipMemsetAsync((char*)c->d_ft_hslot.p + o, 0, std::min<uint64_t>(1ULL << 30, 2 * nbk * 8 - o), c->stream));
	if (n) { hipLaunchKernelGGL(hao_ft_hash_kernel, dim3((unsigned)((n + 255) / 256)), dim3(256), 0, c->stream, c->d_ft_keys.p, c->d_ft_vals.p, n, hb, c->d_ft_hbit.p, c->d_ft_hslot.p); HAO_CHECK_LAUNCH(); }
	return HAO_OK;
}

struct BlkInv { const uint32_t *k; __host__ __device__ uint64_t operator()(uint64_t i) const { return (i > 0 && k[i] < k[i - 1]) ? 1 : 0; } };
struct BlkPair { const uint32_t *k; const uint64_t *v; int xb; __host__ __device__ uint64_t operator()(uint64_t i) const {
	const uint64_t h = v[i]; const uint32_t b = h == UINT64_MAX ? 1u << (12 + xb) : (uint32_t)((h & 4095) << xb | ((h >> 12) & ((1ULL << xb) - 1))); return b != k[i] ? 1 : 0; } };
struct MaxU32 { __host__ __device__ uint64_t operator()(const uint64_t &a, const uint64_t &b) const { return a > b ? a : b; } };
template<typename It, typename Op> static uint64_t hao_dbg_reduce(hao_ctx *c, It it, uint64_t n, Op op)
{
	uint64_t r = 0; size_t tb = 0; (void)c->d_cursor.reserve(2);
	(void)rocprim::reduce(nullptr, tb, it, (uint64_t*)c->d_cursor.p, (uint64_t)0, n, op, c->stream); (void)hao_tmp(c, tb);
	(void)rocprim::reduce(c->d_tmp.p, tb, it, (uint64_t*)c->d_cursor.p, (uint64_t)0, n, op, c->stream);
	(void)hipMemcpy(&r, c->d_cursor.p, 8, hipMemcpyDeviceToHost);
	return r;
}

static int hao_bloom_filter(hao_ctx *c, uint64_t *in, uint64_t *alt, uint64_t n, uint64_t **out, uint64_t **out_alt, uint64_t *n_out)
{
	const int xb = c->opt.bf_shift - 21;
	*out = in; *out_alt = alt; *n_out = 0;
	if (n == 0) return HAO_OK;
	DevBuf<uint32_t> blk, blk2; DevBuf<uint8_t> flag;
	const bool dbg = c->sw.bloom;
	auto now_ = []() { return std::chrono::duration<double>(std::chrono::steady_clock::now().time_since_epoch()).count(); };
	double t_ = now_();
	auto lap = [&](const char *what) { if (dbg) { (void)hipStreamSynchronize(c->stream); const double t1 = now_(); fprintf(stderr, "[bloom] %-14s %8.3f s  (%s)\n", what, t1 - t_, hipGetErrorString(hipGetLastError())); fflush(stderr); t_ = now_(); } };
	if (dbg) fprintf(stderr, "[bloom] n = %llu, xb = %d\n", (unsigned long long)n, xb);
	HIP_TRY(blk.reserve(n + 1)); HIP_TRY(blk2.reserve(n + 1)); HIP_TRY(flag.reserve(n + 1));
	hipLaunchKernelGGL(hao_bf_block_kernel, dim3((unsigned)std::min<uint64_t>((n + 255) / 256, 1u << 20)), dim3(256), 0, c->stream, in, n, xb, blk.p);
	HAO_CHECK_LAUNCH();
	lap("alloc+blockid");
	size_t tb = 0; rocprim::double_buffer<uint32_t> dk(blk.p, blk2.p); rocprim::double_buffer<uint64_t> dv(in, alt);
	HIP_TRY(rocprim::radix_sort_pairs(nullptr, tb, dk, dv, n, 0, 13 + xb, c->stream)); HIP_TRY(hao_tmp(c, tb));
	HIP_TRY(rocprim::radix_sort_pairs(c->d_tmp.p, tb, dk, dv, n, 0, 13 + xb, c->stream));
	lap("sort_pairs");
	if (dbg) {
		const uint64_t inv = hao_dbg_reduce(c, rocprim::make_transform_iterator(rocprim::make_counting_iterator<uint64_t>(0), BlkInv{dk.current()}), n, rocprim::plus<uint64_t>());
		const uint64_t mis = hao_dbg_reduce(c, rocprim::make_transform_iterator(rocprim::make_counting_iterator<uint64_t>(0), BlkPair{dk.current(), dv.current(), xb}), n, rocprim::plus<uint64_t>());
		fprintf(stderr, "[bloom] after the sort: %llu inversions, %llu (key, value) pairs that do not belong together\n", (unsigned long long)inv, (unsigned long long)mis);
		lap("checks");
	}
	{
		const uint64_t max_runs = std::min<uint64_t>(n, (1ULL << (12 + xb)) + 1);
		DevBuf<uint32_t> rk, rl; DevBuf<uint64_t> rs; uint64_t n_runs = 0;
		HIP_TRY(rk.reserve(max_runs + 1)); HIP_TRY(rl.reserve(max_runs + 1)); HIP_TRY(rs.reserve(max_runs + 2)); HIP_TRY(c->d_cursor.reserve(2));
		if (int rc = hao_memset_big(c, flag.p, 0, n)) return rc;
		if (int rc = hao_rle(c, (const uint32_t*)dk.current(), n, rk.p, rl.p, (uint64_t*)c->d_cursor.p)) return rc;
		HIP_TRY(hipMemcpyAsync(&n_runs, c->d_cursor.p, 8, hipMemcpyDeviceToHost, c->stream));
		HIP_TRY(hipStreamSynchronize(c->stream));
		lap("rle");
		auto it = rocprim::make_transform_iterator(rl.p, U32ToU64());
		if (dbg) {
			const uint64_t sum = hao_dbg_reduce(c, it, n_runs, rocprim::plus<uint64_t>()), mx = hao_dbg_reduce(c, it, n_runs, MaxU32());
			fprintf(stderr, "[bloom] runs: %llu (bound %llu), lengths sum to %llu (n = %llu), longest %llu\n", (unsigned long long)n_runs, (unsigned long long)max_runs, (unsigned long long)sum, (unsigned long long)n, (unsigned long long)mx);
			if (n_runs > max_runs) { hao_set_err(c, "bloom replay: more runs than blocks"); return HAO_EUNSUPP; }
		}
		if (int rc = hao_excl_scan_u64(c, it, rs.p, n_runs)) return rc;
		hipLaunchKernelGGL(hao_bf_replay_kernel, dim3((unsigned)((n_runs + 255) / 256)), dim3(256), 0, c->stream, rk.p, rl.p, rs.p, n_runs, dv.current(), xb, flag.p);
		HAO_CHECK_LAUNCH();
		HIP_TRY(hipStreamSynchronize(c->stream));
		lap("replay");
	}
	HIP_TRY(c->d_cursor.reserve(2));
	tb = 0;
	HIP_TRY(rocprim::select(nullptr, tb, dv.current(), flag.p, dv.alternate(), (uint64_t*)c->d_cursor.p, n, c->stream)); HIP_TRY(hao_tmp(c, tb));
	HIP_TRY(rocprim::select(c->d_tmp.p, tb, dv.current(), flag.p, dv.alternate(), (uint64_t*)c->d_cursor.p, n, c->stream));
	HIP_TRY(hipMemcpyAsync(n_out, c->d_cursor.p, 8, hipMemcpyDeviceToHost, c->stream));
	HIP_TRY(hipStreamSynchronize(c->stream));
	*out = dv.alternate(); *out_alt = dv.current();
	lap("select");
	if (dbg) fprintf(stderr, "[bloom] %llu of %llu occurrences reach the count table\n", (unsigned long long)*n_out, (unsigned long long)n);
	return HAO_OK;
}

struct FtPassPred {
	const uint64_t *bnd; int W, low12;
	__host__ __device__ bool operator()(const uint64_t &h) const {
		if (h == UINT64_MAX) return false;
		const uint64_t key = low12 ? (h & 4095) : h;
		for (int d = 0; d < W; ++d) if (key >= bnd[2 * d] && key <= bnd[2 * d + 1]) return true;
		return false;
	}
};
#define HAO_FT_BYTES_PER_SLOT 20.0
#define HAO_FT_BYTES_PER_SLOT_SHARDED 46.0
#define HAO_FT_RUN_BYTES_PER_SLOT 3.0
#define HAO_FT_BYTES_PER_SLOT_BLOOM 10.0
#define HAO_FT_CHUNK_SLOTS (1ULL << 28)
static uint64_t hao_ft_pass_count(hao_ctx *c, uint64_t n_slots, bool sharded, bool bloom)
{
	if (c->sw.ft_passes > 0) return (uint64_t)c->sw.ft_passes;
	size_t fr = 0, tot = 0;
	if (hipMemGetInfo(&fr, &tot) != hipSuccess) { (void)hipGetLastError(); return 1; }
	const double per_slot = (sharded ? HAO_FT_BYTES_PER_SLOT_SHARDED : HAO_FT_BYTES_PER_SLOT) + (bloom ? HAO_FT_BYTES_PER_SLOT_BLOOM : 0.0);
	const double need = per_slot * (double)n_slots + (double)(1ULL << 30), have = 0.9 * (double)fr;
	const uint64_t p_size = (n_slots + (1ULL << 32) - 1) >> 32;
	if (need <= have) return std::max<uint64_t>(1, std::min<uint64_t>(64, p_size));
	const double rest = have - 2.0 * 8.0 * (double)HAO_FT_CHUNK_SLOTS - (double)(2ULL << 30) - HAO_FT_RUN_BYTES_PER_SLOT * (double)n_slots;
	if (rest <= 0) return 64;
	return (uint64_t)std::min<double>(64.0, std::max<double>((double)p_size, std::ceil(per_slot * (double)n_slots / rest)));
}

static int hao_ft_run(hao_ctx *c)
{
	const uint64_t n = c->n_reads; const int k = c->opt.k;
	c->has_ft = false; c->h_ft_keys.clear(); c->h_ft_vals.clear();
	std::vector<uint32_t> slist;
	DevBuf<uint64_t> slots, chunks, kmer_off, kh_chunk_off, kh, kh2;
	uint64_t n_slots = 0, n_chunks = 0, n_real = 0;
	DevBuf<uint64_t> ukeys; DevBuf<uint32_t> ucnt; uint64_t n_unique = 0, *sorted = nullptr;
	const bool sharded = c->comm && c->comm->active();
	const bool bloom = c->opt.bf_shift >= 21;
	uint64_t n_cnt = 0; uint64_t *cnt_in = nullptr, *cnt_alt = nullptr; uint32_t bias = 0;
	uint64_t P = 1, pass_cap = 0;
	std::vector<uint64_t> h_kmer_off, h_chunk_off;
	DevBuf<uint64_t> ch_tmp, ch_sel, d_bnd;
	auto hash_reads = [&](uint64_t a, uint64_t b, uint64_t slot_base, uint64_t chunk_base, uint64_t n_ch, uint64_t n_sl, uint64_t *out, uint64_t *scalar_real) -> int {
		if (scalar_real) *scalar_real = 0;
		const auto s0 = std::lower_bound(slist.begin(), slist.end(), (uint32_t)a), s1 = std::lower_bound(slist.begin(), slist.end(), (uint32_t)b);
		if (s0 != s1) {
			if (int rc = hao_memset_big(c, out, 0xff, n_sl * 8)) return rc;
			HIP_TRY(c->d_cursor.reserve(4)); HIP_TRY(hipMemsetAsync(c->d_cursor.p + 2, 0, 8, c->stream));
			const uint32_t ns = (uint32_t)(s1 - s0);
			hipLaunchKernelGGL(kmer_hash_scalar_kernel, dim3((ns + 63) / 64), dim3(64), 0, c->stream, c->d_packed.p, c->d_pk_off.p, c->d_len.p,
							   c->d_nsite_off.p, c->d_nsite.p, c->d_scalar_list.p + (s0 - slist.begin()), ns, kmer_off.p, (uint64_t)0, k, c->opt.hpc, out - slot_base, c->d_cursor.p + 2);
			HAO_CHECK_LAUNCH();
			if (scalar_real) { HIP_TRY(hipMemcpyAsync(scalar_real, c->d_cursor.p + 2, 8, hipMemcpyDeviceToHost, c->stream)); HIP_TRY(hipStreamSynchronize(c->stream)); }
		}
		if (n_ch) {
			hao_kh_args a_;
			a_.packed = c->d_packed.p; a_.pk_off = c->d_pk_off.p; a_.len = c->d_len.p; a_.tile_off = c->d_tile_off.p; a_.tile_ord = c->d_tile_ord.p; a_.n_runs = c->d_n_runs.p;
			a_.chunk_off = kh_chunk_off.p; a_.scalar_flag = c->d_scalar_flag.p; a_.kmer_off = kmer_off.p; a_.rid_lo = 0; a_.n_sel = n; a_.k = k; a_.hpc = c->opt.hpc; a_.out = out - slot_base; a_.ch0 = chunk_base;
			hipLaunchKernelGGL(kmer_hash_chunk_kernel, dim3((unsigned)n_ch), dim3(256), hao_kh_smem_bytes(k), c->stream, a_);
			HAO_CHECK_LAUNCH();
		}
		return HAO_OK;
	};
	auto local_index = [&]() -> int {
		if (n == 0) { hao_set_err(c, "no reads"); return HAO_EINVAL; }
		if (c->n_bases >= (1ULL << 32) * 16) { hao_set_err(c, "read set too large for one device pass"); return HAO_EUNSUPP; }
		if (int rc = hao_prepare_runs(c, 0, n, false, slist)) return rc;
		HIP_TRY(slots.reserve(n + 2)); HIP_TRY(chunks.reserve(n + 2)); HIP_TRY(kmer_off.reserve(n + 2)); HIP_TRY(kh_chunk_off.reserve(n + 2));
		hipLaunchKernelGGL(hao_kmer_slots_kernel, dim3((unsigned)((n + 256) / 256)), dim3(256), 0, c->stream, c->d_n_runs.p, c->d_scalar_flag.p, c->d_len.p, (uint64_t)0, n, k, slots.p, chunks.p);
		HAO_CHECK_LAUNCH();
		if (int rc = hao_excl_scan_u64(c, slots.p, kmer_off.p, n + 1)) return rc;
		if (int rc = hao_excl_scan_u64(c, chunks.p, kh_chunk_off.p, n + 1)) return rc;
		HIP_TRY(hipMemcpyAsync(&n_slots, kmer_off.p + n, 8, hipMemcpyDeviceToHost, c->stream));
		HIP_TRY(hipMemcpyAsync(&n_chunks, kh_chunk_off.p + n, 8, hipMemcpyDeviceToHost, c->stream));
		HIP_TRY(hipStreamSynchronize(c->stream));
		c->timer.mark("ft_index");
		if (bloom && c->opt.bf_shift - 21 + 12 > 31) { hao_set_err(c, "bf_shift > 40 is not supported"); return HAO_EUNSUPP; }
		return HAO_OK;
	};
	const int index_rc = local_index();
	if (index_rc && !sharded) return index_rc;
	P = index_rc ? 1 : hao_ft_pass_count(c, n_slots, sharded, bloom);
	if (sharded) {
		hao_comm &cm = *c->comm;
		if (int rc = hao_shard_layout_check(c, cm, index_rc)) return rc;
		std::vector<uint64_t> all; if (int rc = hao_comm_allgather_u64(c, cm, P, all, 0)) return rc;
		for (uint64_t v : all) P = std::max(P, v);
	}
	c->ft_passes_used = (int)P;
	auto local_hashes = [&](uint64_t pass) -> int {
		if (P == 1) {
			HIP_TRY(kh.reserve(n_slots + 1)); HIP_TRY(kh2.reserve(n_slots + 1));
			n_real = n_slots;
			uint64_t scalar_real = 0;
			if (int rc = hash_reads(0, n, 0, 0, n_chunks, n_slots, kh.p, &scalar_real)) return rc;
			if (!slist.empty()) { uint64_t scalar_slots = 0; for (uint32_t r : slist) scalar_slots += c->h_len[r]; n_real = n_slots - scalar_slots + scalar_real; }
		} else {
			if (pass == 0) {
				h_kmer_off.resize(n + 1); h_chunk_off.resize(n + 1);
				HIP_TRY(hipMemcpyAsync(h_kmer_off.data(), kmer_off.p, (n + 1) * 8, hipMemcpyDeviceToHost, c->stream));
				HIP_TRY(hipMemcpyAsync(h_chunk_off.data(), kh_chunk_off.p, (n + 1) * 8, hipMemcpyDeviceToHost, c->stream));
				HIP_TRY(hipStreamSynchronize(c->stream));
				const uint64_t all_slots = h_kmer_off[n];
				pass_cap = std::min<uint64_t>(all_slots, all_slots / P + all_slots / (4 * P) + (1ULL << 20));
				uint64_t biggest = 0; for (uint64_t r = 0; r < n; ++r) biggest = std::max(biggest, h_kmer_off[r + 1] - h_kmer_off[r]);
				const uint64_t chs = std::min<uint64_t>(all_slots, std::max<uint64_t>(c->sw.ft_chunk_slots ? (uint64_t)c->sw.ft_chunk_slots : HAO_FT_CHUNK_SLOTS, biggest));
				HIP_TRY(ch_tmp.reserve_exact(chs + 1)); HIP_TRY(ch_sel.reserve_exact(chs + 1)); HIP_TRY(kh.reserve_exact(pass_cap + 1)); HIP_TRY(kh2.reserve_exact(pass_cap + 1));
				HIP_TRY(d_bnd.reserve(2 * 4096 + 2)); HIP_TRY(c->d_cursor.reserve(4));
			}
			const int W = sharded ? c->comm->world : 1; std::vector<uint64_t> bnd(2 * (size_t)W);
			for (int d = 0; d < W; ++d) {
				unsigned __int128 lo, hi;
				if (!bloom) { lo = d == 0 ? 0 : (((unsigned __int128)d << 64) / (unsigned)W); hi = d + 1 == W ? ((unsigned __int128)1 << 64) : (((unsigned __int128)(d + 1) << 64) / (unsigned)W); }
				else { lo = ((uint64_t)d * 4096 + W - 1) / W; hi = d + 1 == W ? 4096 : ((uint64_t)(d + 1) * 4096 + W - 1) / W; }
				const unsigned __int128 span = hi - lo, a_ = lo + span * pass / P, b_ = lo + span * (pass + 1) / P;
				if (a_ == b_) { bnd[2 * d] = 1; bnd[2 * d + 1] = 0; } else { bnd[2 * d] = (uint64_t)a_; bnd[2 * d + 1] = (uint64_t)(b_ - 1); }
			}
			HIP_TRY(hipMemcpyAsync(d_bnd.p, bnd.data(), bnd.size() * 8, hipMemcpyHostToDevice, c->stream));
			const FtPassPred pred{d_bnd.p, W, bloom ? 1 : 0};
			uint64_t cnt = 0; const uint64_t chs = ch_tmp.cap - 1;
			for (uint64_t a = 0; a < n; ) {
				uint64_t b = a + 1; while (b < n && h_kmer_off[b + 1] - h_kmer_off[a] <= chs) ++b;
				const uint64_t sl = h_kmer_off[b] - h_kmer_off[a], nch = h_chunk_off[b] - h_chunk_off[a];
				if (sl) {
					if (int rc = hash_reads(a, b, h_kmer_off[a], h_chunk_off[a], nch, sl, ch_tmp.p, nullptr)) return rc;
					size_t tb = 0; uint64_t sel = 0;
					HIP_TRY(rocprim::select(nullptr, tb, ch_tmp.p, ch_sel.p, (uint64_t*)c->d_cursor.p, (size_t)sl, pred, c->stream)); HIP_TRY(hao_tmp(c, tb));
					HIP_TRY(rocprim::select(c->d_tmp.p, tb, ch_tmp.p, ch_sel.p, (uint64_t*)c->d_cursor.p, (size_t)sl, pred, c->stream));
					HIP_TRY(hipMemcpyAsync(&sel, c->d_cursor.p, 8, hipMemcpyDeviceToHost, c->stream));
					HIP_TRY(hipStreamSynchronize(c->stream));
					if (cnt + sel > pass_cap) { hao_set_err(c, "ha_ft_gen: a hash-range pass holds more k-mer occurrences than its buffer (set HAO_FT_PASSES higher)"); return HAO_ENOMEM; }
					if (sel) HIP_TRY(hipMemcpyAsync(kh.p + cnt, ch_sel.p, sel * 8, hipMemcpyDeviceToDevice, c->stream));
					cnt += sel;
				}
				a = b;
			}
			HIP_TRY(hipStreamSynchronize(c->stream));
			n_slots = cnt; n_real = cnt;
		}
		c->timer.mark("ft_hash");
		n_cnt = n_slots; cnt_in = kh.p; cnt_alt = kh2.p; bias = 0;
		if (bloom) {
			if (!sharded) { if (int rc = hao_bloom_filter(c, kh.p, kh2.p, n_slots, &cnt_in, &cnt_alt, &n_cnt)) return rc; }
			bias = 1;
			c->timer.mark("ft_bloom");
		}
		return HAO_OK;
	};
	DevBuf<uint64_t> all_keys; DevBuf<uint32_t> all_cnt; uint64_t all_unique = 0; int64_t all_hist[HAO_N_COUNTS];
	memset(all_hist, 0, sizeof(all_hist));
	for (uint64_t pass = 0; pass < P; ++pass) {
	const int hash_rc = local_hashes(pass);
	if (hash_rc && !sharded) return hash_rc;
	if (!sharded) {
		if (int rc = hao_sort_rle_hist(c, cnt_in, cnt_alt, n_cnt, ukeys, ucnt, &n_unique, c->ft_hist, &sorted, bias)) return rc;
		if (!bloom && n_real < n_slots && n_unique) { --n_unique; c->ft_hist[std::min<uint64_t>(n_slots - n_real, HAO_MAX_COUNT)] -= 1; }
	} else {
		hao_comm &cm = *c->comm; const int W = cm.world;
		uint64_t *loc = kh.p; uint64_t n_loc = n_real;
		std::vector<uint64_t> tg(W), cut(W + 1, 0), scnt(W, 0), sdisp(W, 0), rcnt;
		DevBuf<uint64_t> dt, dc, rv, rv2;
		auto local_partition = [&]() -> int {
			if (hash_rc) return hash_rc;
			HIP_TRY(dt.reserve(W + 1)); HIP_TRY(dc.reserve(W + 1));
			if (!bloom) {
				if (n_slots) {
					size_t tb = 0; rocprim::double_buffer<uint64_t> db(kh.p, kh2.p);
					HIP_TRY(rocprim::radix_sort_keys(nullptr, tb, db, n_slots, 0, 64, c->stream)); HIP_TRY(hao_tmp(c, tb));
					HIP_TRY(rocprim::radix_sort_keys(c->d_tmp.p, tb, db, n_slots, 0, 64, c->stream));
					loc = db.current();
				}
				for (int d = 0; d < W; ++d) tg[d] = d == 0 ? 0 : (uint64_t)(((unsigned __int128)d << 64) / (unsigned)W);
				HIP_TRY(hipMemcpyAsync(dt.p, tg.data(), 8 * W, hipMemcpyHostToDevice, c->stream));
				hipLaunchKernelGGL(hao_lower_bound_kernel, dim3((W + 63) / 64), dim3(64), 0, c->stream, loc, n_real, dt.p, W, dc.p);
				HAO_CHECK_LAUNCH();
			} else {
				if (n_slots) {
					HIP_TRY(c->d_cursor.reserve(4)); size_t tb = 0;
					HIP_TRY(rocprim::select(nullptr, tb, kh.p, kh2.p, (uint64_t*)c->d_cursor.p, n_slots, NotSentinel(), c->stream)); HIP_TRY(hao_tmp(c, tb));
					HIP_TRY(rocprim::select(c->d_tmp.p, tb, kh.p, kh2.p, (uint64_t*)c->d_cursor.p, n_slots, NotSentinel(), c->stream));
					HIP_TRY(hipMemcpyAsync(&n_loc, c->d_cursor.p, 8, hipMemcpyDeviceToHost, c->stream));
					HIP_TRY(hipStreamSynchronize(c->stream));
					tb = 0; rocprim::double_buffer<uint64_t> db(kh2.p, kh.p);
					HIP_TRY(rocprim::radix_sort_keys(nullptr, tb, db, n_loc, 0, 12, c->stream)); HIP_TRY(hao_tmp(c, tb));
					HIP_TRY(rocprim::radix_sort_keys(c->d_tmp.p, tb, db, n_loc, 0, 12, c->stream));
					loc = db.current();
				}
				for (int d = 0; d < W; ++d) tg[d] = ((uint64_t)d * 4096 + W - 1) / W;
				HIP_TRY(hipMemcpyAsync(dt.p, tg.data(), 8 * W, hipMemcpyHostToDevice, c->stream));
				hipLaunchKernelGGL(hao_lower_bound_low12_kernel, dim3((W + 63) / 64), dim3(64), 0, c->stream, loc, n_loc, dt.p, W, dc.p);
				HAO_CHECK_LAUNCH();
			}
			HIP_TRY(hipMemcpyAsync(cut.data(), dc.p, 8 * W, hipMemcpyDeviceToHost, c->stream));
			HIP_TRY(hipStreamSynchronize(c->stream));
			cut[W] = n_loc;
			for (int d = 0; d < W; ++d) { sdisp[d] = cut[d]; scnt[d] = cut[d + 1] - cut[d]; }
			return HAO_OK;
		};
		if (int rc = hao_comm_exchange_counts(c, cm, scnt, rcnt, local_partition())) return rc;
		uint64_t n_recv = 0; for (int d = 0; d < W; ++d) n_recv += rcnt[d];
		auto local_recv_bufs = [&]() -> int { if (P == 1) { if (loc == kh.p) kh2.release(); else kh.release(); } HIP_TRY(rv.reserve(n_recv + 1)); return HAO_OK; };
		if (int rc = hao_comm_agree(c, cm, local_recv_bufs())) return rc;
		if (int rc = hao_comm_alltoallv_u64(c, cm, loc, scnt, sdisp, rv.p, rcnt)) return rc;
		HIP_TRY(hipStreamSynchronize(c->stream));
		c->timer.mark("ft_exchange");
		auto local_count = [&]() -> int {
			if (P == 1) { kh.release(); kh2.release(); }
			HIP_TRY(rv2.reserve(n_recv + 1));
			uint64_t *ci = rv.p, *ca = rv2.p, n_ci = n_recv;
			if (bloom) { if (int rc = hao_bloom_filter(c, rv.p, rv2.p, n_recv, &ci, &ca, &n_ci)) return rc; }
			return hao_sort_rle_hist(c, ci, ca, n_ci, ukeys, ucnt, &n_unique, c->ft_hist, &sorted, bias);
		};
		if (int rc = hao_comm_allreduce_i64(c, cm, c->ft_hist, HAO_N_COUNTS, local_count())) return rc;
	}
	if (P > 1) {
		if (all_unique + n_unique + 1 > all_keys.cap) {
			const uint64_t want = std::max<uint64_t>((all_unique + n_unique) * (pass + 1 < P ? 2 : 1) + 64, (n_unique + 64) * (P - pass));
			DevBuf<uint64_t> nk_; DevBuf<uint32_t> nc_; HIP_TRY(nk_.reserve_exact(want)); HIP_TRY(nc_.reserve_exact(want));
			if (all_unique) { HIP_TRY(hipMemcpyAsync(nk_.p, all_keys.p, all_unique * 8, hipMemcpyDeviceToDevice, c->stream)); HIP_TRY(hipMemcpyAsync(nc_.p, all_cnt.p, all_unique * 4, hipMemcpyDeviceToDevice, c->stream)); HIP_TRY(hipStreamSynchronize(c->stream)); }
			std::swap(all_keys, nk_); std::swap(all_cnt, nc_);
		}
		if (n_unique) { HIP_TRY(hipMemcpyAsync(all_keys.p + all_unique, ukeys.p, n_unique * 8, hipMemcpyDeviceToDevice, c->stream)); HIP_TRY(hipMemcpyAsync(all_cnt.p + all_unique, ucnt.p, n_unique * 4, hipMemcpyDeviceToDevice, c->stream)); HIP_TRY(hipStreamSynchronize(c->stream)); }
		all_unique += n_unique;
		for (int i = 0; i < HAO_N_COUNTS; ++i) all_hist[i] += c->ft_hist[i];
	}
	}
	if (P > 1) {
		kh.release(); kh2.release(); ch_tmp.release(); ch_sel.release(); ukeys.release(); ucnt.release();
		if (bloom && all_unique) {
			DevBuf<uint64_t> k2; DevBuf<uint32_t> c2; HIP_TRY(k2.reserve_exact(all_unique + 1)); HIP_TRY(c2.reserve_exact(all_unique + 1));
			size_t tb = 0; rocprim::double_buffer<uint64_t> dk(all_keys.p, k2.p); rocprim::double_buffer<uint32_t> dv(all_cnt.p, c2.p);
			HIP_TRY(rocprim::radix_sort_pairs(nullptr, tb, dk, dv, all_unique, 0, 64, c->stream)); HIP_TRY(hao_tmp(c, tb));
			HIP_TRY(rocprim::radix_sort_pairs(c->d_tmp.p, tb, dk, dv, all_unique, 0, 64, c->stream));
			HIP_TRY(hipStreamSynchronize(c->stream));
			if (dk.current() != all_keys.p) std::swap(all_keys, k2);
			if (dv.current() != all_cnt.p) std::swap(all_cnt, c2);
		}
		std::swap(ukeys, all_keys); std::swap(ucnt, all_cnt); n_unique = all_unique;
		memcpy(c->ft_hist, all_hist, sizeof(all_hist));
	}
	c->timer.mark("ft_count");
	kh.release(); kh2.release();
	c->ft_peak_hom = hao_find_peaks(c->ft_hist, HAO_N_COUNTS, c->opt.min_hist_cnt, &c->ft_peak_het, hao_prior_hom(c));
	int cutoff = (int)(c->ft_peak_hom * c->opt.high_factor);
	if (cutoff > HAO_MAX_COUNT - 1) cutoff = HAO_MAX_COUNT - 1;
	c->ft_cutoff = cutoff;
	DevBuf<uint32_t> kcnt; uint64_t n_kept = 0;
	const int keep_rc = hao_keep_runs(c, ukeys.p, ucnt.p, n_unique, cutoff, HAO_MAX_COUNT, c->d_ft_keys, nullptr, kcnt, &n_kept, nullptr);
	if (keep_rc && !sharded) return keep_rc;
	ukeys.release(); ucnt.release(); c->w_flag.release(); c->w_kpos.release(); c->w_ustart.release();
	if (sharded) {
		hao_comm &cm = *c->comm; std::vector<uint64_t> cnts;
		if (int rc = hao_comm_allgather_u64(c, cm, n_kept, cnts, keep_rc)) return rc;
		uint64_t tot = 0; for (uint64_t v : cnts) tot += v;
		DevBuf<uint64_t> gk; DevBuf<uint32_t> gc;
		auto local_bufs = [&]() -> int { HIP_TRY(gk.reserve(tot + 1)); HIP_TRY(gc.reserve(tot + 1)); return HAO_OK; };
		if (int rc = hao_comm_agree(c, cm, local_bufs())) return rc;
		if (int rc = hao_comm_allgatherv(c, cm, c->d_ft_keys.p, n_kept, 8, gk.p, cnts)) return rc;
		if (int rc = hao_comm_allgatherv(c, cm, kcnt.p, n_kept, 4, gc.p, cnts)) return rc;
		HIP_TRY(hipStreamSynchronize(c->stream));
		if (bloom && tot) {
			DevBuf<uint64_t> gk2; DevBuf<uint32_t> gc2; HIP_TRY(gk2.reserve(tot + 1)); HIP_TRY(gc2.reserve(tot + 1));
			size_t tb = 0; rocprim::double_buffer<uint64_t> dk(gk.p, gk2.p); rocprim::double_buffer<uint32_t> dv(gc.p, gc2.p);
			HIP_TRY(rocprim::radix_sort_pairs(nullptr, tb, dk, dv, tot, 0, 64, c->stream)); HIP_TRY(hao_tmp(c, tb));
			HIP_TRY(rocprim::radix_sort_pairs(c->d_tmp.p, tb, dk, dv, tot, 0, 64, c->stream));
			HIP_TRY(hipStreamSynchronize(c->stream));
			if (dk.current() != gk.p) std::swap(gk, gk2);
			if (dv.current() != gc.p) std::swap(gc, gc2);
		}
		std::swap(c->d_ft_keys, gk); std::swap(kcnt, gc);
		n_kept = tot;
	}
	int max_cnt = c->opt.max_kmer_cnt;
	if (max_cnt > HAO_MAX_COUNT - 1) max_cnt = HAO_MAX_COUNT - 1;
	if (max_cnt > INT16_MAX - 1) max_cnt = INT16_MAX - 1;
	c->h_ft_keys.resize(n_kept); c->h_ft_vals.resize(n_kept);
	std::vector<uint32_t> hc(n_kept);
	if (n_kept) {
		HIP_TRY(hipMemcpy(c->h_ft_keys.data(), c->d_ft_keys.p, n_kept * 8, hipMemcpyDeviceToHost));
		HIP_TRY(hipMemcpy(hc.data(), kcnt.p, n_kept * 4, hipMemcpyDeviceToHost));
	}
	for (uint64_t i = 0; i < n_kept; ++i) c->h_ft_vals[i] = (int)hc[i] > max_cnt ? INT32_MAX : (int32_t)hc[i];
	HIP_TRY(c->d_ft_vals.reserve(n_kept + 1)); HIP_TRY(c->d_ft_keys.reserve(n_kept + 1));
	if (n_kept) HIP_TRY(hipMemcpyAsync(c->d_ft_vals.p, c->h_ft_vals.data(), n_kept * 4, hipMemcpyHostToDevice, c->stream));
	if (int rc = hao_build_bucket(c, c->d_ft_keys.p, n_kept, 16, c->d_ft_bucket)) return rc;
	if (int rc = hao_ft_build_hash(c, n_kept)) return rc;
	HIP_TRY(hipStreamSynchronize(c->stream));
	kcnt.release(); slots.release(); chunks.release(); kmer_off.release(); kh_chunk_off.release();
	c->has_ft = true;
	{
		int mx = (int)(c->ft_peak_hom * c->opt.high_factor + .499);
		c->hom_cov = c->ft_peak_hom;
		if (c->max_n_chain < mx) c->max_n_chain = mx;
	}
	c->timer.mark("ft_table");
	return HAO_OK;
}

static inline uint64_t hao_sort40_cap(uint64_t m) { return std::max<uint64_t>(1 << 16, m >> 10); }
static int hao_index_sort(hao_ctx *c, const uint64_t *x, uint64_t *sx, uint32_t *oi, uint32_t *oi2, uint64_t m, bool sort40)
{
	hipLaunchKernelGGL(hao_iota_kernel, dim3((unsigned)((m + 255) / 256)), dim3(256), 0, c->stream, oi, m); HAO_CHECK_LAUNCH();
	const int b0 = sort40 ? HAO_SORT40_LOWBITS : 0;
	size_t tb = 0;
	HIP_TRY(rocprim::radix_sort_pairs(nullptr, tb, x, sx, oi, oi2, m, b0, 64, c->stream)); HIP_TRY(hao_tmp(c, tb));
	HIP_TRY(rocprim::radix_sort_pairs(c->d_tmp.p, tb, x, sx, oi, oi2, m, b0, 64, c->stream));
	if (sort40) {
		const uint64_t cap = hao_sort40_cap(m), tcap = 64 * cap;
		HIP_TRY(c->w_s40_list.reserve(cap)); HIP_TRY(c->w_s40_x.reserve(tcap)); HIP_TRY(c->w_s40_o.reserve(tcap)); HIP_TRY(c->w_s40_cnt.reserve(4));
		HIP_TRY(hipMemsetAsync(c->w_s40_cnt.p, 0, 32, c->stream));
		hipLaunchKernelGGL(hao_sort40_mark_kernel, dim3((unsigned)((m + 255) / 256)), dim3(256), 0, c->stream, sx, m, c->w_s40_list.p, c->w_s40_cnt.p, cap); HAO_CHECK_LAUNCH();
		hipLaunchKernelGGL(hao_sort40_fix_kernel, dim3((unsigned)cap), dim3(64), 0, c->stream, sx, oi2, m, c->w_s40_list.p, c->w_s40_cnt.p, cap, c->w_s40_x.p, c->w_s40_o.p, tcap); HAO_CHECK_LAUNCH();
		if (int rc = hao_peek(c, c->w_s40_cnt.p, 3, PK_SORT40)) return rc;
	}
	return HAO_OK;
}

static int hao_pt_run(hao_ctx *c)
{
	const uint64_t n = c->n_reads;
	c->has_pt = false; c->h_ix_valid = false; c->h_ix_mz_off.clear();
	const bool sharded = c->comm && c->comm->active();
	auto local_sketch = [&]() -> int {
		if (n == 0) { hao_set_err(c, "no reads"); return HAO_EINVAL; }
		if (int rc = hao_sketch_run(c, 0, n, c->has_ft, c->opt.sample_dist, 1)) return rc;
		std::swap(c->d_ix_mz_x, c->d_mz_x); std::swap(c->d_ix_mz_info, c->d_mz_info); std::swap(c->d_ix_mz_off, c->d_mz_off);
		HIP_TRY(c->d_mz_x.reserve_exact(c->d_ix_mz_x.cap)); HIP_TRY(c->d_mz_info.reserve_exact(c->d_ix_mz_info.cap)); HIP_TRY(c->d_mz_off.reserve_exact(c->d_ix_mz_off.cap));
		c->ix_n_mz = c->sk_total; c->sk_n = 0;
		return HAO_OK;
	};
	const int sk_rc = local_sketch();
	if (sk_rc && !sharded) return sk_rc;
	DevBuf<uint64_t> &ukeys = c->w_ukeys; DevBuf<uint32_t> &ucnt = c->w_ucnt; uint64_t n_unique = 0;
	memset(c->pt_hist, 0, sizeof(c->pt_hist));
	auto rle_hist = [&](const uint64_t *sorted, uint64_t cnt) -> int {
		n_unique = 0;
		if (!cnt) return HAO_OK;
		HIP_TRY(ukeys.reserve(cnt + 1)); HIP_TRY(ucnt.reserve(cnt + 1)); HIP_TRY(c->d_cursor.reserve(2));
		if (int rc = hao_rle(c, sorted, cnt, ukeys.p, ucnt.p, (uint64_t*)c->d_cursor.p)) return rc;
		HIP_TRY(hipMemcpyAsync(&n_unique, c->d_cursor.p, 8, hipMemcpyDeviceToHost, c->stream));
		HIP_TRY(hipStreamSynchronize(c->stream));
		DevBuf<unsigned long long> &dh = c->w_hist; HIP_TRY(dh.reserve(HAO_N_COUNTS)); HIP_TRY(hipMemsetAsync(dh.p, 0, HAO_N_COUNTS * 8, c->stream));
		unsigned nb = (unsigned)std::min<uint64_t>((n_unique + 255) / 256, 2048);
		if (nb) hipLaunchKernelGGL(hao_count_hist_kernel, dim3(nb), dim3(256), 0, c->stream, ucnt.p, n_unique, dh.p);
		HAO_CHECK_LAUNCH();
		HIP_TRY(hipMemcpyAsync(c->pt_hist, dh.p, HAO_N_COUNTS * 8, hipMemcpyDeviceToHost, c->stream));
		HIP_TRY(hipStreamSynchronize(c->stream));
		return HAO_OK;
	};
	auto peaks_and_range = [&](int *hi_out) {
		int het = -1;
		c->hom_cov = hao_find_peaks(c->pt_hist, HAO_N_COUNTS, c->opt.min_hist_cnt, &het, hao_prior_hom(c)); c->het_cov = het;
		int hi;
		if (c->has_ft) hi = HAO_MAX_COUNT - 1;
		else { hi = (int)(c->hom_cov * c->opt.high_factor); if (hi > HAO_MAX_COUNT - 1) hi = HAO_MAX_COUNT - 1; }
		*hi_out = hi;
	};
	c->lk_valid = false;
	if (!sharded) {
		const uint64_t m = c->ix_n_mz;
		if (m >= (1ULL << 32)) { hao_set_err(c, "more than 2^32 minimizers on one device"); return HAO_EUNSUPP; }
		const uint64_t pad = c->ix_pad = c->sw.ix_pad;
		HIP_TRY(c->d_ix_sx.reserve(m + 1)); HIP_TRY(c->d_ix_sinfo.reserve(m + pad + 8)); HIP_TRY(c->w_oi.reserve(m + 1)); HIP_TRY(c->w_oi2.reserve(m + 1));
		HIP_TRY(c->w_runid.reserve(m + 1)); HIP_TRY(c->d_ix_lk.reserve(m + 1));
		bool sort40 = m >= c->sw.sort40_min;
		for (;;) {
			if (m) { if (int rc = hao_index_sort(c, c->d_ix_mz_x.p, c->d_ix_sx.p, c->w_oi.p, c->w_oi2.p, m, sort40)) return rc; }
			c->ix_n_sorted = m;
			c->timer.mark("pt_sort");
			if (int rc = rle_hist(c->d_ix_sx.p, m)) return rc;
			if (m && sort40) {
				c->s40_runs = c->peeked(PK_SORT40);
				if (c->s40_runs > hao_sort40_cap(m) || c->peeked(PK_SORT40, 2)) { sort40 = false; continue; }
			}
			break;
		}
		c->timer.mark("pt_count");
		int hi; peaks_and_range(&hi);
		if (int rc = hao_keep_runs(c, ukeys.p, ucnt.p, n_unique, 2, hi, c->d_ix_keys, &c->d_ix_start, c->d_ix_cnt, &c->ix_n_keys, &c->ix_n_pos)) return rc;
		if (m) {
			auto heads = rocprim::make_transform_iterator(rocprim::make_counting_iterator<uint64_t>(0), RunHead32{c->d_ix_sx.p});
			size_t tb = 0;
			HIP_TRY(rocprim::inclusive_scan(nullptr, tb, heads, c->w_runid.p, m, rocprim::plus<uint32_t>(), c->stream)); HIP_TRY(hao_tmp(c, tb));
			HIP_TRY(rocprim::inclusive_scan(c->d_tmp.p, tb, heads, c->w_runid.p, m, rocprim::plus<uint32_t>(), c->stream));
			if (m >= c->sw.sort40_min) {
				int nb = 1; while ((1ULL << nb) < m) ++nb;
				const int b0 = nb > 8 ? nb - 8 : 0;
				HIP_TRY(c->w_lkv2.reserve(m + 1));
				hipLaunchKernelGGL(hao_index_gather_kernel, dim3((unsigned)((m + 255) / 256)), dim3(256), 0, c->stream, m, c->w_oi2.p, c->w_runid.p, ucnt.p, c->w_ustart.p, 2, hi,
								   c->d_ix_mz_info.p, c->d_ix_sinfo.p + pad, c->d_ix_sx.p, pad);
				HAO_CHECK_LAUNCH();
				size_t tb2 = 0;
				HIP_TRY(rocprim::radix_sort_pairs(nullptr, tb2, c->w_oi2.p, c->w_oi.p, c->d_ix_sx.p, c->w_lkv2.p, m, b0, nb, c->stream)); HIP_TRY(hao_tmp(c, tb2));
				HIP_TRY(rocprim::radix_sort_pairs(c->d_tmp.p, tb2, c->w_oi2.p, c->w_oi.p, c->d_ix_sx.p, c->w_lkv2.p, m, b0, nb, c->stream));
				hipLaunchKernelGGL(hao_scatter_u64_kernel, dim3((unsigned)((m + 255) / 256)), dim3(256), 0, c->stream, c->w_lkv2.p, c->w_oi.p, m, c->d_ix_lk.p);
				HAO_CHECK_LAUNCH();
			} else {
				hipLaunchKernelGGL(hao_index_finish_kernel, dim3((unsigned)((m + 255) / 256)), dim3(256), 0, c->stream, m, c->w_oi2.p, c->w_runid.p, ucnt.p, c->w_ustart.p, 2, hi,
								   c->d_ix_mz_info.p, c->d_ix_sinfo.p + pad, c->d_ix_lk.p, pad);
				HAO_CHECK_LAUNCH();
			}
			if (pad && c->ix_n_keys) { hipLaunchKernelGGL(hao_add_const_kernel, dim3((unsigned)((c->ix_n_keys + 255) / 256)), dim3(256), 0, c->stream, c->d_ix_start.p, c->ix_n_keys, pad); HAO_CHECK_LAUNCH(); }
		}
		c->lk_valid = true;
		c->timer.mark("pt_lookup");
	} else {
		hao_comm &cm = *c->comm; const int W = cm.world;
		if (int rc = hao_shard_layout_check(c, cm, sk_rc)) return rc;
		const uint64_t ml = c->ix_n_mz;
		DevBuf<uint64_t> lsx, lsi, dt, dc, rx, ri, px, pi, lkr, lkl; DevBuf<uint32_t> ai, ai2; const uint32_t *lperm = nullptr;
		std::vector<uint64_t> tg(W), cut(W + 1, 0), scnt(W, 0), sdisp(W, 0), rcnt;
		auto local_group = [&]() -> int {
			HIP_TRY(lsx.reserve(ml + 1)); HIP_TRY(lsi.reserve(ml + 1));
			if (ml) {
				DevBuf<uint32_t> &ok = c->w_ok, &ok2 = c->w_ok2, &oi = c->w_oi, &oi2 = c->w_oi2;
				HIP_TRY(ok.reserve(ml + 1)); HIP_TRY(ok2.reserve(ml + 1)); HIP_TRY(oi.reserve(ml + 1)); HIP_TRY(oi2.reserve(ml + 1));
				hipLaunchKernelGGL(hao_owner_key_kernel, dim3((unsigned)((ml + 255) / 256)), dim3(256), 0, c->stream, c->d_ix_mz_x.p, ml, ok.p, oi.p);
				HAO_CHECK_LAUNCH();
				size_t tb = 0; rocprim::double_buffer<uint32_t> dk(ok.p, ok2.p), dv(oi.p, oi2.p);
				HIP_TRY(rocprim::radix_sort_pairs(nullptr, tb, dk, dv, ml, 0, 16, c->stream)); HIP_TRY(hao_tmp(c, tb));
				HIP_TRY(rocprim::radix_sort_pairs(c->d_tmp.p, tb, dk, dv, ml, 0, 16, c->stream));
				hipLaunchKernelGGL(hao_gather2_kernel, dim3((unsigned)((ml + 255) / 256)), dim3(256), 0, c->stream, dv.current(), c->d_ix_mz_x.p, c->d_ix_mz_info.p, ml, lsx.p, lsi.p);
				HAO_CHECK_LAUNCH();
				lperm = dv.current();
			}
			for (int d = 0; d < W; ++d) tg[d] = (((uint64_t)d * 65536 + W - 1) / W) << 48;
			HIP_TRY(dt.reserve(W + 1)); HIP_TRY(dc.reserve(W + 1));
			HIP_TRY(hipMemcpyAsync(dt.p, tg.data(), 8 * W, hipMemcpyHostToDevice, c->stream));
			hipLaunchKernelGGL(hao_lower_bound_kernel, dim3((W + 63) / 64), dim3(64), 0, c->stream, lsx.p, ml, dt.p, W, dc.p);
			HAO_CHECK_LAUNCH();
			HIP_TRY(hipMemcpyAsync(cut.data(), dc.p, 8 * W, hipMemcpyDeviceToHost, c->stream));
			HIP_TRY(hipStreamSynchronize(c->stream));
			cut[W] = ml;
			for (int d = 0; d < W; ++d) { sdisp[d] = cut[d]; scnt[d] = cut[d + 1] - cut[d]; }
			return HAO_OK;
		};
		if (int rc = hao_comm_exchange_counts(c, cm, scnt, rcnt, local_group())) return rc;
		uint64_t n_recv = 0; for (int d = 0; d < W; ++d) n_recv += rcnt[d];
		auto local_recv_bufs = [&]() -> int { HIP_TRY(rx.reserve(n_recv + 1)); HIP_TRY(ri.reserve(n_recv + 1)); HIP_TRY(px.reserve(n_recv + 1)); HIP_TRY(pi.reserve(n_recv + 1)); return HAO_OK; };
		if (int rc = hao_comm_agree(c, cm, local_recv_bufs())) return rc;
		if (int rc = hao_comm_alltoallv2_u64(c, cm, lsx.p, lsi.p, scnt, sdisp, rx.p, ri.p, rcnt)) return rc;
		HIP_TRY(hipStreamSynchronize(c->stream));
		c->timer.mark("pt_alltoall");
		auto local_count = [&]() -> int {
			if (n_recv >= (1ULL << 32)) { hao_set_err(c, "more than 2^32 minimizers in one hash partition"); return HAO_EUNSUPP; }
			HIP_TRY(ai.reserve(n_recv + 1)); HIP_TRY(ai2.reserve(n_recv + 1));
			if (n_recv) {
				hipLaunchKernelGGL(hao_iota_kernel, dim3((unsigned)((n_recv + 255) / 256)), dim3(256), 0, c->stream, ai.p, n_recv); HAO_CHECK_LAUNCH();
				size_t tb = 0;
				HIP_TRY(rocprim::radix_sort_pairs(nullptr, tb, rx.p, px.p, ai.p, ai2.p, n_recv, 0, 64, c->stream)); HIP_TRY(hao_tmp(c, tb));
				HIP_TRY(rocprim::radix_sort_pairs(c->d_tmp.p, tb, rx.p, px.p, ai.p, ai2.p, n_recv, 0, 64, c->stream));
			}
			c->timer.mark("pt_sort");
			return rle_hist(px.p, n_recv);
		};
		if (int rc = hao_comm_allreduce_i64(c, cm, c->pt_hist, HAO_N_COUNTS, local_count())) return rc;
		c->timer.mark("pt_count");
		int hi; peaks_and_range(&hi);
		DevBuf<uint64_t> pk, pst; DevBuf<uint32_t> pc; uint64_t nk_p = 0, np_p = 0;
		const int keep_rc = hao_keep_runs(c, ukeys.p, ucnt.p, n_unique, 2, hi, pk, &pst, pc, &nk_p, &np_p);
		std::vector<uint64_t> part(W), nks(W), nps(W), trip;
		{ const uint64_t mine[3] = { n_recv, nk_p, np_p };
		  if (int rc = hao_comm_allgather_u64n(c, cm, mine, 3, trip, keep_rc)) return rc;
		  for (int r = 0; r < W; ++r) { part[r] = trip[3 * r]; nks[r] = trip[3 * r + 1]; nps[r] = trip[3 * r + 2]; } }
		uint64_t m = 0, base = 0, nk = 0, np = 0;
		for (int r = 0; r < W; ++r) { if (r < cm.rank) base += part[r]; m += part[r]; nk += nks[r]; np += nps[r]; }
		const uint64_t pad = c->ix_pad = c->sw.ix_pad; base += pad;
		{
			auto local_lk = [&]() -> int {
				HIP_TRY(lkr.reserve(n_recv + 1)); HIP_TRY(lkl.reserve(ml + 1)); HIP_TRY(c->w_runid.reserve(n_recv + 1)); HIP_TRY(c->d_ix_lk.reserve(ml + 1));
				if (n_recv) {
					auto heads = rocprim::make_transform_iterator(rocprim::make_counting_iterator<uint64_t>(0), RunHead32{px.p});
					size_t tb = 0;
					HIP_TRY(rocprim::inclusive_scan(nullptr, tb, heads, c->w_runid.p, n_recv, rocprim::plus<uint32_t>(), c->stream)); HIP_TRY(hao_tmp(c, tb));
					HIP_TRY(rocprim::inclusive_scan(c->d_tmp.p, tb, heads, c->w_runid.p, n_recv, rocprim::plus<uint32_t>(), c->stream));
					hipLaunchKernelGGL(hao_index_finish_kernel, dim3((unsigned)((n_recv + 255) / 256)), dim3(256), 0, c->stream, n_recv, ai2.p, c->w_runid.p, ucnt.p, c->w_ustart.p, 2, hi,
									   ri.p, pi.p, lkr.p, base);
					HAO_CHECK_LAUNCH();
				}
				return HAO_OK;
			};
			if (int rc = hao_comm_agree(c, cm, local_lk())) return rc;
			std::vector<uint64_t> rdisp(W, 0), back;
			for (int d = 1; d < W; ++d) rdisp[d] = rdisp[d - 1] + rcnt[d - 1];
			if (int rc = hao_comm_alltoallv_u64(c, cm, lkr.p, rcnt, rdisp, lkl.p, scnt)) return rc;
			if (ml) { hipLaunchKernelGGL(hao_scatter_u64_kernel, dim3((unsigned)((ml + 255) / 256)), dim3(256), 0, c->stream, lkl.p, lperm, ml, c->d_ix_lk.p); HAO_CHECK_LAUNCH(); }
			HIP_TRY(hipStreamSynchronize(c->stream));
			c->lk_valid = true;
			c->timer.mark("pt_lookup");
		}
		uint64_t maxm = 0, maxk = 0; for (int r = 0; r < W; ++r) { maxm = std::max(maxm, part[r]); maxk = std::max(maxk, nks[r]); }
		const size_t o_key = (size_t)maxm * 8, o_st = o_key + (size_t)maxk * 8, o_cnt = o_st + (size_t)maxk * 8, slot = (o_cnt + (size_t)maxk * 4 + 15) & ~(size_t)15;
		auto local_slot = [&]() -> int {
			if (nk_p) { hipLaunchKernelGGL(hao_add_const_kernel, dim3((unsigned)((nk_p + 255) / 256)), dim3(256), 0, c->stream, pst.p, nk_p, base); HAO_CHECK_LAUNCH(); }
			HIP_TRY(c->d_ix_sinfo.reserve(m + pad + 8));
			HIP_TRY(c->d_ix_keys.reserve(nk + 1)); HIP_TRY(c->d_ix_start.reserve(nk + 1)); HIP_TRY(c->d_ix_cnt.reserve(nk + 1));
			HIP_TRY(cm.ag_tmp.reserve(slot * W + 16));
			char *mine = cm.ag_tmp.p + slot * cm.rank;
			if (n_recv) HIP_TRY(hipMemcpyAsync(mine, pi.p, n_recv * 8, hipMemcpyDeviceToDevice, c->stream));
			if (nk_p) {
				HIP_TRY(hipMemcpyAsync(mine + o_key, pk.p, nk_p * 8, hipMemcpyDeviceToDevice, c->stream));
				HIP_TRY(hipMemcpyAsync(mine + o_st, pst.p, nk_p * 8, hipMemcpyDeviceToDevice, c->stream));
				HIP_TRY(hipMemcpyAsync(mine + o_cnt, pc.p, nk_p * 4, hipMemcpyDeviceToDevice, c->stream));
			}
			return HAO_OK;
		};
		if (int rc = hao_comm_agree(c, cm, local_slot())) return rc;
		if (int rc = hao_comm_allgather_fixed(c, cm, cm.ag_tmp.p, slot)) return rc;
		uint64_t dm = pad, dk = 0;
		for (int r = 0; r < W; ++r) {
			const char *sr = cm.ag_tmp.p + slot * r;
			if (part[r]) HIP_TRY(hipMemcpyAsync(c->d_ix_sinfo.p + dm, sr, part[r] * 8, hipMemcpyDeviceToDevice, c->stream));
			if (nks[r]) {
				HIP_TRY(hipMemcpyAsync(c->d_ix_keys.p + dk, sr + o_key, nks[r] * 8, hipMemcpyDeviceToDevice, c->stream));
				HIP_TRY(hipMemcpyAsync(c->d_ix_start.p + dk, sr + o_st, nks[r] * 8, hipMemcpyDeviceToDevice, c->stream));
				HIP_TRY(hipMemcpyAsync(c->d_ix_cnt.p + dk, sr + o_cnt, nks[r] * 4, hipMemcpyDeviceToDevice, c->stream));
			}
			dm += part[r]; dk += nks[r];
		}
		HIP_TRY(hipStreamSynchronize(c->stream));
		c->ix_n_sorted = m; c->ix_n_keys = nk; c->ix_n_pos = np;
		lsx.release(); lsi.release(); rx.release(); ri.release(); px.release(); pi.release(); lkr.release(); lkl.release(); ai.release(); ai2.release(); pk.release(); pst.release(); pc.release(); dt.release(); dc.release();
		c->timer.mark("pt_allgather");
	}
	int bits = 16; while ((1ULL << bits) < c->ix_n_keys / 2 && bits < 26) ++bits;
	if (int rc = hao_build_bucket(c, c->d_ix_keys.p, c->ix_n_keys, bits, c->d_ix_bucket)) return rc;
	c->ix_bucket_bits = bits;
	c->h_ix_mz_off.resize(n + 1);
	HIP_TRY(hipMemcpyAsync(c->h_ix_mz_off.data(), c->d_ix_mz_off.p, (n + 1) * 8, hipMemcpyDeviceToHost, c->stream));
	HIP_TRY(hipStreamSynchronize(c->stream));
	if (!c->has_ft) { int mx = (int)(c->hom_cov * c->opt.high_factor + .499); if (c->max_n_chain < mx) c->max_n_chain = mx; }
	c->has_pt = true;
	c->timer.mark("pt_table");
	return HAO_OK;
}

static hao_pt_dev hao_pt_view(hao_ctx *c)
{
	hao_pt_dev p; p.keys = c->d_ix_keys.p; p.start = c->d_ix_start.p; p.cnt = c->d_ix_cnt.p; p.bucket = c->d_ix_bucket.p; p.sinfo = c->d_ix_sinfo.p;
	p.n_keys = c->ix_n_keys; p.bshift = 64 - c->ix_bucket_bits;
	return p;
}

static int hao_pt_download(hao_ctx *c)
{
	if (c->h_ix_valid) return HAO_OK;
	const uint64_t nk = c->ix_n_keys;
	std::vector<uint64_t> start(nk); std::vector<uint32_t> cnt(nk); std::vector<uint64_t> sinfo(c->ix_n_sorted);
	c->h_ix_keys.resize(nk); c->h_ix_off.resize(nk + 1); c->h_ix_pos.resize(c->ix_n_pos);
	if (nk) {
		HIP_TRY(hipMemcpy(c->h_ix_keys.data(), c->d_ix_keys.p, nk * 8, hipMemcpyDeviceToHost));
		HIP_TRY(hipMemcpy(start.data(), c->d_ix_start.p, nk * 8, hipMemcpyDeviceToHost));
		HIP_TRY(hipMemcpy(cnt.data(), c->d_ix_cnt.p, nk * 4, hipMemcpyDeviceToHost));
	}
	if (c->ix_n_sorted) HIP_TRY(hipMemcpy(sinfo.data(), c->d_ix_sinfo.p + c->ix_pad, c->ix_n_sorted * 8, hipMemcpyDeviceToHost));
	uint64_t o = 0;
	for (uint64_t i = 0; i < nk; ++i) { c->h_ix_off[i] = o; memcpy(c->h_ix_pos.data() + o, sinfo.data() + (start[i] - c->ix_pad), (size_t)cnt[i] * 8); o += cnt[i]; }
	c->h_ix_off[nk] = o;
	c->h_ix_valid = true;
	return HAO_OK;
}
```

Baseline: 179.6 million.

## Cache sketch run plan across sketch and k-mer counting passes

Moves the per-read tile offsets, HPC run index, scalar flags/lists and chunk offsets into a SketchPlan keyed by read range, generation and k/w/hpc, so the host-side plan building, H2D uploads, hpc_index kernel and the synchronisations are skipped when the same range is sketched again. The k-mer counting path now shares this plan, using separate N-site flags and lists in place of its own prepare-runs call. A debug print of host time before the sketch kernel is added. The cost is extra device memory kept alive for the plan, and correctness depends on the generation counter being bumped whenever the reads change.

```diff
diff --git a/hifiasm_amd/csrc/hao_capi.hip b/hifiasm_amd/csrc/hao_capi.hip
--- a/hifiasm_amd/csrc/hao_capi.hip
+++ b/hifiasm_amd/csrc/hao_capi.hip
@@ -78,7 +78,7 @@
 				  const uint64_t *nsite_off, const uint32_t *nsite)
 {
 	if (!c || !packed || !pk_off || !len) return HAO_EINVAL;
-	HAO_NOT_ON_VIEW(c, "hao_set_reads"); ++c->index_gen;
+	HAO_NOT_ON_VIEW(c, "hao_set_reads"); ++c->index_gen; ++c->reads_gen;
 	hao_gather_drop(c);
 	if (n_reads >= (1ULL << 28)) { hao_set_err(c, "more than 2^28 reads (htab.cpp:765)"); return HAO_EUNSUPP; }
 	HIP_TRY(hipSetDevice(c->device));
@@ -114,7 +114,7 @@
 int hao_set_shard(hao_ctx *c, uint64_t rid_base, uint64_t n_total, const uint32_t *all_len)
 {
 	if (!c || !all_len || rid_base + c->n_reads > n_total) return HAO_EINVAL;
-	HAO_NOT_ON_VIEW(c, "hao_set_shard"); ++c->index_gen;
+	HAO_NOT_ON_VIEW(c, "hao_set_shard"); ++c->index_gen; ++c->reads_gen;
 	hao_gather_drop(c);
 	if (n_total >= (1ULL << 28)) { hao_set_err(c, "more than 2^28 reads (htab.cpp:765)"); return HAO_EUNSUPP; }
 	for (uint64_t i = 0; i < c->n_reads; ++i) if (all_len[rid_base + i] != c->h_len[i]) { hao_set_err(c, "all_len disagrees with the local read lengths"); return HAO_EINVAL; }
diff --git a/hifiasm_amd/csrc/hao_ctx.hpp b/hifiasm_amd/csrc/hao_ctx.hpp
--- a/hifiasm_amd/csrc/hao_ctx.hpp
+++ b/hifiasm_amd/csrc/hao_ctx.hpp
@@ -62,7 +62,7 @@
 };
 
 struct hao_switches {
-	bool seedphase = false, qcphase = false, dp_stats = false, selphase = false, dltime = false, bloom = false;
+	bool seedphase = false, qcphase = false, dp_stats = false, selphase = false, dltime = false, bloom = false, skhost = false;
 	bool seq_chain = false, dp_seqtail = false, dp_nospec = false, dp_serial = false, seq_prune = false, seed_noql = false, al_coop = false;
 	long long sk_gcap = -1, exc_cap = -1, ft_chunk_slots = 0; unsigned long long gather_chunk = 64ULL << 20, al_slice = 4ULL << 30, ix_pad = 0, sort40_min = 1ULL << 23; int fc_raw_every = 0, exc_every = 0; bool qmz_raw = false, arena_probe = false;
 	int arena_numa = 3, seed_merge_maxn = 24000, seed_lds_ratio = 120, ft_passes = 0, seed_lds = 1;
@@ -78,7 +78,7 @@
 	}
 	void load() {
 		if (const char *v = getenv("HAO_DBG_PRINT")) {
-			seedphase = in_list(v, "seed"); qcphase = in_list(v, "qc"); dp_stats = in_list(v, "dp"); selphase = in_list(v, "sel"); dltime = in_list(v, "dl"); bloom = in_list(v, "bloom"); hao_dbg_sync = in_list(v, "sync");
+			seedphase = in_list(v, "seed"); qcphase = in_list(v, "qc"); dp_stats = in_list(v, "dp"); selphase = in_list(v, "sel"); dltime = in_list(v, "dl"); bloom = in_list(v, "bloom"); skhost = in_list(v, "sk"); hao_dbg_sync = in_list(v, "sync");
 		}
 		if (const char *v = getenv("HAO_DBG_FORCE")) {
 			seq_chain = in_list(v, "seq_chain");
@@ -177,6 +177,14 @@
 	DevBuf<uint64_t> *wl_woff; DevBuf<hao_rs_win> *wl_wins; DevBuf<uint64_t> *wl_cigoff; DevBuf<uint16_t> *wl_cig;
 };
 
+struct SketchPlan {
+	DevBuf<uint64_t> d_tile_off, d_chunk_off; DevBuf<uint32_t> d_tile_ord, d_n_runs, d_scalar_list, d_n_list, d_unit_rid; DevBuf<uint8_t> d_scalar_flag, d_n_flag;
+	std::vector<uint32_t> slist, nlist; uint64_t n_chunks = 0, nb = 0;
+	bool valid = false; uint64_t lo = 0, hi = 0, gen = 0; int k = 0, w = 0, hpc = 0, variant = 0, chunk = 0;
+	bool serves(uint64_t lo_, uint64_t hi_, uint64_t gen_, int k_, int w_, int hpc_, int variant_, int chunk_) const
+	{ return valid && lo == lo_ && hi == hi_ && gen == gen_ && k == k_ && w == w_ && hpc == hpc_ && variant == variant_ && chunk == chunk_; }
+};
+
 struct hao_ctx {
 	int device = 0; hao_opt_t opt; std::string err; hipStream_t stream = nullptr; hao_switches sw;
 	hao_ctx *owner = nullptr; uint64_t index_gen = 0, attached_gen = 0;
@@ -194,8 +202,8 @@
 	DevBuf<uint32_t> d_ft_hbit; DevBuf<unsigned long long> d_ft_hslot; int ft_hbits = 0;
 	int max_n_chain = 100, hom_cov = -1, het_cov = -1;
 	uint64_t sk_lo = 0, sk_n = 0, sk_total = 0; bool sk_is_index = false;
-	DevBuf<uint64_t> d_tile_off; DevBuf<uint32_t> d_tile_ord, d_n_runs, d_tot_l; DevBuf<uint64_t> d_chunk_off, d_chunk_cnt64;
-	DevBuf<uint8_t> d_scalar_flag; DevBuf<uint32_t> d_scalar_list, d_unit_rid;
+	SketchPlan plan; uint64_t reads_gen = 0;
+	DevBuf<uint32_t> d_tot_l; DevBuf<uint64_t> d_chunk_cnt64;
 	DevBuf<uint64_t> d_pool_x, d_pool_info; DevBuf<uint32_t> d_pool_ord; DevBuf<unsigned long long> d_cursor; DevBuf<int> d_err;
 	DevBuf<uint64_t> d_chunk_base, d_chunk_dst; DevBuf<uint32_t> d_chunk_cnt;
 	DevBuf<uint64_t> d_g_x, d_g_info; DevBuf<uint32_t> d_g_ord; DevBuf<uint64_t> d_g_off; DevBuf<uint32_t> d_new_n; DevBuf<uint64_t> d_new_n64;
diff --git a/hifiasm_amd/csrc/hao_gather.hpp b/hifiasm_amd/csrc/hao_gather.hpp
--- a/hifiasm_amd/csrc/hao_gather.hpp
+++ b/hifiasm_amd/csrc/hao_gather.hpp
@@ -114,7 +114,7 @@
 	if (c->owner) { hao_set_err(c, "hao_dist_gather_reads: not on an attached batch context (hao_attach)"); return HAO_EINVAL; }
 	if (!hao_is_sharded(c) || c->gs_valid) return HAO_OK;
 	HIP_TRY(hipSetDevice(c->device));
-	++c->index_gen;
+	++c->index_gen; ++c->reads_gen;
 	const int rc = hao_gather_reads_run(c);
 	if (rc) hao_gather_drop(c);
 	return rc;
diff --git a/hifiasm_amd/csrc/hao_pipeline.hpp b/hifiasm_amd/csrc/hao_pipeline.hpp
--- a/hifiasm_amd/csrc/hao_pipeline.hpp
+++ b/hifiasm_amd/csrc/hao_pipeline.hpp
@@ -28,56 +28,83 @@
 	return f;
 }
 
-static int hao_sketch_run(hao_ctx *c, uint64_t lo, uint64_t hi, int use_ft, int sample_dist, int stamp_rid)
+enum { HAO_SKV_UNIT, HAO_SKV_WAVE, HAO_SKV_CHUNK };
+static inline int hao_sk_variant(int k, int w, int *chunk)
 {
-	const uint64_t n_sel = hi - lo; const int k = c->opt.k, w = c->opt.w;
-	const bool unit_variant = w == 51 && k == 51;
-	const bool wave_variant = w == 51 && k + 7 <= 64;
-	const int chunk = unit_variant ? hao_sk3<51, 51>::MW : (wave_variant ? hao_sk2<51>::CHUNK : HAO_SK_CHUNK);
-	c->sk_lo = lo; c->sk_n = n_sel; c->sk_total = 0;
-	HIP_TRY(c->d_mz_off.reserve(n_sel + 2));
-	if (n_sel == 0) { HIP_TRY(hipMemsetAsync(c->d_mz_off.p, 0, 8, c->stream)); return HAO_OK; }
-	std::vector<uint64_t> tile_off(n_sel + 1); std::vector<uint8_t> flag(n_sel); std::vector<uint32_t> slist; uint64_t nb = 0;
+	if (w == 51 && k == 51) { *chunk = hao_sk3<51, 51>::MW; return HAO_SKV_UNIT; }
+	if (w == 51 && k + 7 <= 64) { *chunk = hao_sk2<51>::CHUNK; return HAO_SKV_WAVE; }
+	*chunk = HAO_SK_CHUNK; return HAO_SKV_CHUNK;
+}
+
+static int hao_plan_ensure(hao_ctx *c, uint64_t lo, uint64_t hi, bool marks)
+{
+	SketchPlan &P = c->plan;
+	const uint64_t n_sel = hi - lo; const int k = c->opt.k, w = c->opt.w, hpc = c->opt.hpc;
+	int chunk = 0; const int variant = hao_sk_variant(k, w, &chunk); const bool unit_variant = variant == HAO_SKV_UNIT;
+	if (P.serves(lo, hi, c->reads_gen, k, w, hpc, variant, chunk)) { if (marks) { c->timer.mark("sk_h2d"); c->timer.mark("sk_index"); } return HAO_OK; }
+	P.valid = false;
+	std::vector<uint64_t> tile_off(n_sel + 1); std::vector<uint8_t> flag(n_sel), nflag(n_sel); uint64_t nb = 0;
+	P.slist.clear(); P.nlist.clear();
 	const bool even_k = (k & 1) == 0;
 	for (uint64_t r = 0; r < n_sel; ++r) {
 		uint32_t L = c->h_len[lo + r];
 		tile_off[r] = r == 0 ? 0 : tile_off[r - 1] + (c->h_len[lo + r - 1] + HAO_SK_TILE - 1) / HAO_SK_TILE + 1;
 		bool hasn = c->has_n && c->h_nsite_off[lo + r + 1] > c->h_nsite_off[lo + r];
-		flag[r] = (hasn || even_k) ? 1 : 0;
-		if (flag[r]) slist.push_back((uint32_t)r);
+		flag[r] = (hasn || even_k) ? 1 : 0; nflag[r] = hasn ? 1 : 0;
+		if (flag[r]) P.slist.push_back((uint32_t)r);
+		if (hasn) P.nlist.push_back((uint32_t)r);
 		nb += L;
 	}
 	tile_off[n_sel] = tile_off[n_sel - 1] + (c->h_len[hi - 1] + HAO_SK_TILE - 1) / HAO_SK_TILE + 1;
-	HIP_TRY(c->d_tile_off.reserve(n_sel + 1)); HIP_TRY(c->d_tile_ord.reserve(tile_off[n_sel] + 1)); HIP_TRY(c->d_n_runs.reserve(n_sel + 1));
-	HIP_TRY(c->d_tot_l.reserve(n_sel + 1)); HIP_TRY(c->d_scalar_flag.reserve(n_sel + 1)); HIP_TRY(c->d_scalar_list.reserve(slist.size() + 1));
-	HIP_TRY(c->d_chunk_off.reserve(n_sel + 2)); HIP_TRY(c->d_chunk_cnt64.reserve(n_sel + 2)); HIP_TRY(c->d_cursor.reserve(2)); HIP_TRY(c->d_err.reserve(2));
-	HIP_TRY(hipMemcpyAsync(c->d_tile_off.p, tile_off.data(), (n_sel + 1) * 8, hipMemcpyHostToDevice, c->stream));
-	HIP_TRY(hipMemcpyAsync(c->d_scalar_flag.p, flag.data(), n_sel, hipMemcpyHostToDevice, c->stream));
-	if (!slist.empty()) HIP_TRY(hipMemcpyAsync(c->d_scalar_list.p, slist.data(), slist.size() * 4, hipMemcpyHostToDevice, c->stream));
-	c->timer.mark("sk_h2d");
+	HIP_TRY(P.d_tile_off.reserve(n_sel + 1)); HIP_TRY(P.d_tile_ord.reserve(tile_off[n_sel] + 1)); HIP_TRY(P.d_n_runs.reserve(n_sel + 1));
+	HIP_TRY(P.d_scalar_flag.reserve(n_sel + 1)); HIP_TRY(P.d_scalar_list.reserve(P.slist.size() + 1)); HIP_TRY(P.d_n_flag.reserve(n_sel + 1)); HIP_TRY(P.d_n_list.reserve(P.nlist.size() + 1));
+	HIP_TRY(P.d_chunk_off.reserve(n_sel + 2)); HIP_TRY(c->d_chunk_cnt64.reserve(n_sel + 2));
+	HIP_TRY(hipMemcpyAsync(P.d_tile_off.p, tile_off.data(), (n_sel + 1) * 8, hipMemcpyHostToDevice, c->stream));
+	HIP_TRY(hipMemcpyAsync(P.d_scalar_flag.p, flag.data(), n_sel, hipMemcpyHostToDevice, c->stream));
+	HIP_TRY(hipMemcpyAsync(P.d_n_flag.p, nflag.data(), n_sel, hipMemcpyHostToDevice, c->stream));
+	if (!P.slist.empty()) HIP_TRY(hipMemcpyAsync(P.d_scalar_list.p, P.slist.data(), P.slist.size() * 4, hipMemcpyHostToDevice, c->stream));
+	if (!P.nlist.empty()) HIP_TRY(hipMemcpyAsync(P.d_n_list.p, P.nlist.data(), P.nlist.size() * 4, hipMemcpyHostToDevice, c->stream));
+	if (marks) c->timer.mark("sk_h2d");
 	hipLaunchKernelGGL(hpc_index_kernel, dim3((unsigned)((n_sel + 3) / 4)), dim3(256), 0, c->stream, c->d_packed.p, c->d_pk_off.p, c->d_len.p,
-					   c->d_tile_off.p, c->d_tile_ord.p, c->d_n_runs.p, lo, n_sel, c->opt.hpc, unit_variant ? c->d_scalar_flag.p : (uint8_t*)nullptr);
+					   P.d_tile_off.p, P.d_tile_ord.p, P.d_n_runs.p, lo, n_sel, hpc, unit_variant ? P.d_scalar_flag.p : (uint8_t*)nullptr);
 	HAO_CHECK_LAUNCH();
-	hipLaunchKernelGGL(hao_chunk_count_kernel, dim3((unsigned)((n_sel + 256) / 256)), dim3(256), 0, c->stream, c->d_n_runs.p, c->d_scalar_flag.p, n_sel, k, chunk, c->d_chunk_cnt64.p);
+	hipLaunchKernelGGL(hao_chunk_count_kernel, dim3((unsigned)((n_sel + 256) / 256)), dim3(256), 0, c->stream, P.d_n_runs.p, P.d_scalar_flag.p, n_sel, k, chunk, c->d_chunk_cnt64.p);
 	HAO_CHECK_LAUNCH();
-	if (int rc = hao_excl_scan_u64(c, c->d_chunk_cnt64.p, c->d_chunk_off.p, n_sel + 1)) return rc;
-	HIP_TRY(hipMemcpyAsync(c->d_tot_l.p, c->d_n_runs.p, n_sel * 4, hipMemcpyDeviceToDevice, c->stream));
+	if (int rc = hao_excl_scan_u64(c, c->d_chunk_cnt64.p, P.d_chunk_off.p, n_sel + 1)) return rc;
 	uint64_t n_chunks = 0;
-	HIP_TRY(hipMemcpyAsync(&n_chunks, c->d_chunk_off.p + n_sel, 8, hipMemcpyDeviceToHost, c->stream));
-	if (unit_variant) HIP_TRY(hipMemcpyAsync(flag.data(), c->d_scalar_flag.p, n_sel, hipMemcpyDeviceToHost, c->stream));
+	HIP_TRY(hipMemcpyAsync(&n_chunks, P.d_chunk_off.p + n_sel, 8, hipMemcpyDeviceToHost, c->stream));
+	if (unit_variant) HIP_TRY(hipMemcpyAsync(flag.data(), P.d_scalar_flag.p, n_sel, hipMemcpyDeviceToHost, c->stream));
 	HIP_TRY(hipStreamSynchronize(c->stream));
 	if (unit_variant) {
-		const size_t n0 = slist.size(); slist.clear();
-		for (uint64_t r = 0; r < n_sel; ++r) if (flag[r]) slist.push_back((uint32_t)r);
-		if (slist.size() != n0) { HIP_TRY(c->d_scalar_list.reserve(slist.size() + 1)); HIP_TRY(hipMemcpyAsync(c->d_scalar_list.p, slist.data(), slist.size() * 4, hipMemcpyHostToDevice, c->stream)); }
-	}
-	c->timer.mark("sk_index");
-	HIP_TRY(c->d_chunk_base.reserve(n_chunks + 1)); HIP_TRY(c->d_chunk_cnt.reserve(n_chunks + 1)); HIP_TRY(c->d_chunk_dst.reserve(n_chunks + 2));
-	if (unit_variant) {
-		HIP_TRY(c->d_unit_rid.reserve(n_chunks + 1));
-		hipLaunchKernelGGL(hao_unit_rid_kernel, dim3((unsigned)((n_sel + 255) / 256)), dim3(256), 0, c->stream, c->d_chunk_off.p, n_sel, c->d_unit_rid.p);
+		const size_t n0 = P.slist.size(); P.slist.clear();
+		for (uint64_t r = 0; r < n_sel; ++r) if (flag[r]) P.slist.push_back((uint32_t)r);
+		if (P.slist.size() != n0) {
+			HIP_TRY(P.d_scalar_list.reserve(P.slist.size() + 1)); HIP_TRY(hipMemcpyAsync(P.d_scalar_list.p, P.slist.data(), P.slist.size() * 4, hipMemcpyHostToDevice, c->stream));
+			HIP_TRY(hipStreamSynchronize(c->stream));
+		}
+		HIP_TRY(P.d_unit_rid.reserve(n_chunks + 1));
+		hipLaunchKernelGGL(hao_unit_rid_kernel, dim3((unsigned)((n_sel + 255) / 256)), dim3(256), 0, c->stream, P.d_chunk_off.p, n_sel, P.d_unit_rid.p);
 		HAO_CHECK_LAUNCH();
 	}
+	if (marks) c->timer.mark("sk_index");
+	P.n_chunks = n_chunks; P.nb = nb;
+	P.lo = lo; P.hi = hi; P.gen = c->reads_gen; P.k = k; P.w = w; P.hpc = hpc; P.variant = variant; P.chunk = chunk; P.valid = true;
+	return HAO_OK;
+}
+
+static int hao_sketch_run(hao_ctx *c, uint64_t lo, uint64_t hi, int use_ft, int sample_dist, int stamp_rid)
+{
+	const uint64_t n_sel = hi - lo; const int k = c->opt.k, w = c->opt.w;
+	int chunk = 0; const int variant = hao_sk_variant(k, w, &chunk); (void)chunk;
+	const bool unit_variant = variant == HAO_SKV_UNIT, wave_variant = variant == HAO_SKV_WAVE;
+	c->sk_lo = lo; c->sk_n = n_sel; c->sk_total = 0;
+	HIP_TRY(c->d_mz_off.reserve(n_sel + 2));
+	if (n_sel == 0) { HIP_TRY(hipMemsetAsync(c->d_mz_off.p, 0, 8, c->stream)); return HAO_OK; }
+	if (int rc = hao_plan_ensure(c, lo, hi, true)) return rc;
+	const SketchPlan &P = c->plan; const std::vector<uint32_t> &slist = P.slist; const uint64_t n_chunks = P.n_chunks, nb = P.nb;
+	HIP_TRY(c->d_tot_l.reserve(n_sel + 1)); HIP_TRY(c->d_cursor.reserve(2)); HIP_TRY(c->d_err.reserve(2));
+	HIP_TRY(hipMemcpyAsync(c->d_tot_l.p, P.d_n_runs.p, n_sel * 4, hipMemcpyDeviceToDevice, c->stream));
+	HIP_TRY(c->d_chunk_base.reserve(n_chunks + 1)); HIP_TRY(c->d_chunk_cnt.reserve(n_chunks + 1)); HIP_TRY(c->d_chunk_dst.reserve(n_chunks + 2));
 	if (!slist.empty()) { HIP_TRY(c->d_ring.reserve(slist.size() * 256 * sizeof(hao_cand))); HIP_TRY(c->d_ringord.reserve(slist.size() * 256)); HIP_TRY(c->d_cnt_ws.reserve(slist.size() + 1)); }
 	const size_t smem = hao_sk_smem_bytes(w, k);
 	const uint64_t pool_static = unit_variant ? n_chunks * SK3_SLOT : 0;
@@ -90,7 +117,7 @@
 		HIP_TRY(hipMemsetAsync(c->d_chunk_cnt.p, 0, (n_chunks + 1) * 4, c->stream));
 		if (!slist.empty()) {
 			sa.packed = c->d_packed.p; sa.pk_off = c->d_pk_off.p; sa.len = c->d_len.p; sa.nsite_off = c->has_n ? c->d_nsite_off.p : nullptr; sa.nsite = c->has_n ? c->d_nsite.p : nullptr;
-			sa.chunk_off = c->d_chunk_off.p; sa.scalar_flag = c->d_scalar_flag.p; sa.scalar_list = c->d_scalar_list.p; sa.n_scalar = (uint32_t)slist.size();
+			sa.chunk_off = P.d_chunk_off.p; sa.scalar_flag = P.d_scalar_flag.p; sa.scalar_list = P.d_scalar_list.p; sa.n_scalar = (uint32_t)slist.size();
 			sa.rid_lo = lo; sa.k = k; sa.w = w; sa.hpc = c->opt.hpc; sa.use_ft = use_ft; sa.ft = hao_ft_view(c);
 			sa.ring_ws = (hao_cand*)c->d_ring.p; sa.ringord_ws = c->d_ringord.p;
 			sa.pool_x = c->d_pool_x.p; sa.pool_info = c->d_pool_info.p; sa.pool_ord = c->d_pool_ord.p; sa.pool_cursor = c->d_cursor.p; sa.pool_cap = cap;
@@ -98,11 +125,13 @@
 			hipLaunchKernelGGL(sketch_scalar_kernel, dim3((unsigned)((slist.size() + 63) / 64)), dim3(64), 0, c->stream, sa);
 			HAO_CHECK_LAUNCH();
 		}
+		if (c->sw.skhost && attempt == 0 && !c->timer.host_t.empty())
+			fprintf(stderr, "[sk] %.3f ms of host time in front of the sketch kernel (%llu reads)\n", (StageTimer::now() - c->timer.host_t[0]) * 1e3, (unsigned long long)n_sel);
 		hao_sk_args a;
-		a.packed = c->d_packed.p; a.pk_off = c->d_pk_off.p; a.len = c->d_len.p; a.tile_off = c->d_tile_off.p; a.tile_ord = c->d_tile_ord.p; a.n_runs = c->d_n_runs.p;
-		a.chunk_off = c->d_chunk_off.p; a.scalar_flag = c->d_scalar_flag.p; a.rid_lo = lo; a.n_sel = n_sel; a.k = k; a.w = w; a.hpc = c->opt.hpc; a.ft = hao_ft_view(c);
+		a.packed = c->d_packed.p; a.pk_off = c->d_pk_off.p; a.len = c->d_len.p; a.tile_off = P.d_tile_off.p; a.tile_ord = P.d_tile_ord.p; a.n_runs = P.d_n_runs.p;
+		a.chunk_off = P.d_chunk_off.p; a.scalar_flag = P.d_scalar_flag.p; a.rid_lo = lo; a.n_sel = n_sel; a.k = k; a.w = w; a.hpc = c->opt.hpc; a.ft = hao_ft_view(c);
 		a.pool_x = c->d_pool_x.p; a.pool_info = c->d_pool_info.p; a.pool_ord = c->d_pool_ord.p; a.pool_cursor = c->d_cursor.p; a.pool_cap = cap;
-		a.chunk_base = c->d_chunk_base.p; a.chunk_cnt = c->d_chunk_cnt.p; a.err = c->d_err.p; a.pool_static = pool_static; a.unit_rid = c->d_unit_rid.p; a.n_units = n_chunks;
+		a.chunk_base = c->d_chunk_base.p; a.chunk_cnt = c->d_chunk_cnt.p; a.err = c->d_err.p; a.pool_static = pool_static; a.unit_rid = P.d_unit_rid.p; a.n_units = n_chunks;
 		if (unit_variant) {
 			if (use_ft && a.ft.n > 0) hipLaunchKernelGGL((sketch_unit_kernel<true, 51, 51>), dim3((unsigned)((n_chunks + 3) / 4)), dim3(256), 0, c->stream, a);
 			else hipLaunchKernelGGL((sketch_unit_kernel<false, 51, 51>), dim3((unsigned)((n_chunks + 3) / 4)), dim3(256), 0, c->stream, a);
@@ -120,12 +149,12 @@
 		if (!slist.empty()) { sa.pass = 1; hipLaunchKernelGGL(sketch_scalar_kernel, dim3((unsigned)((slist.size() + 63) / 64)), dim3(64), 0, c->stream, sa); HAO_CHECK_LAUNCH(); }
 		const bool thin = use_ft && a.ft.n > 0 && sample_dist > w;
 		HIP_TRY(c->d_g_off.reserve(n_sel + 2)); HIP_TRY(c->d_mz_x.reserve(gcap + 1)); HIP_TRY(c->d_mz_info.reserve(gcap + 1));
-		hipLaunchKernelGGL(sketch_read_off_kernel, dim3((unsigned)((n_sel + 256) / 256)), dim3(256), 0, c->stream, c->d_chunk_off.p, c->d_chunk_dst.p, n_sel, c->d_g_off.p);
+		hipLaunchKernelGGL(sketch_read_off_kernel, dim3((unsigned)((n_sel + 256) / 256)), dim3(256), 0, c->stream, P.d_chunk_off.p, c->d_chunk_dst.p, n_sel, c->d_g_off.p);
 		HAO_CHECK_LAUNCH();
 		if (!thin) {
 			HIP_TRY(hipMemcpyAsync(c->d_mz_off.p, c->d_g_off.p, (n_sel + 1) * 8, hipMemcpyDeviceToDevice, c->stream));
 			hipLaunchKernelGGL(sketch_gather_finish_kernel, dim3((unsigned)((n_sel + 3) / 4)), dim3(256), 0, c->stream, c->d_pool_x.p, c->d_pool_info.p, c->d_chunk_base.p, c->d_chunk_cnt.p,
-							   c->d_chunk_dst.p, c->d_chunk_off.p, lo + c->rid_base, n_sel, stamp_rid, c->d_mz_x.p, c->d_mz_info.p, gcap, c->d_err.p);
+							   c->d_chunk_dst.p, P.d_chunk_off.p, lo + c->rid_base, n_sel, stamp_rid, c->d_mz_x.p, c->d_mz_info.p, gcap, c->d_err.p);
 			HAO_CHECK_LAUNCH();
 			c->timer.mark("sk_gather");
 		} else {
diff --git a/hifiasm_amd/csrc/hao_tables.hpp b/hifiasm_amd/csrc/hao_tables.hpp
--- a/hifiasm_amd/csrc/hao_tables.hpp
+++ b/hifiasm_amd/csrc/hao_tables.hpp
@@ -45,30 +45,6 @@
 {
 	uint64_t i = (uint64_t)blockIdx.x * blockDim.x + threadIdx.x;
 	if (i < n) cnt[i] = off[i + 1] - off[i];
-}
-
-static int hao_prepare_runs(hao_ctx *c, uint64_t lo, uint64_t hi, bool force_scalar_all, std::vector<uint32_t> &slist)
-{
-	const uint64_t n_sel = hi - lo;
-	std::vector<uint64_t> tile_off(n_sel + 1); std::vector<uint8_t> flag(n_sel);
-	slist.clear();
-	for (uint64_t r = 0; r < n_sel; ++r) {
-		tile_off[r] = r == 0 ? 0 : tile_off[r - 1] + (c->h_len[lo + r - 1] + HAO_SK_TILE - 1) / HAO_SK_TILE + 1;
-		bool hasn = c->has_n && c->h_nsite_off[lo + r + 1] > c->h_nsite_off[lo + r];
-		flag[r] = (hasn || force_scalar_all) ? 1 : 0;
-		if (flag[r]) slist.push_back((uint32_t)r);
-	}
-	tile_off[n_sel] = tile_off[n_sel - 1] + (c->h_len[hi - 1] + HAO_SK_TILE - 1) / HAO_SK_TILE + 1;
-	HIP_TRY(c->d_tile_off.reserve(n_sel + 1)); HIP_TRY(c->d_tile_ord.reserve(tile_off[n_sel] + 1)); HIP_TRY(c->d_n_runs.reserve(n_sel + 1));
-	HIP_TRY(c->d_scalar_flag.reserve(n_sel + 1)); HIP_TRY(c->d_scalar_list.reserve(slist.size() + 1));
-	HIP_TRY(hipMemcpyAsync(c->d_tile_off.p, tile_off.data(), (n_sel + 1) * 8, hipMemcpyHostToDevice, c->stream));
-	HIP_TRY(hipMemcpyAsync(c->d_scalar_flag.p, flag.data(), n_sel, hipMemcpyHostToDevice, c->stream));
-	if (!slist.empty()) HIP_TRY(hipMemcpyAsync(c->d_scalar_list.p, slist.data(), slist.size() * 4, hipMemcpyHostToDevice, c->stream));
-	hipLaunchKernelGGL(hpc_index_kernel, dim3((unsigned)((n_sel + 3) / 4)), dim3(256), 0, c->stream, c->d_packed.p, c->d_pk_off.p, c->d_len.p,
-					   c->d_tile_off.p, c->d_tile_ord.p, c->d_n_runs.p, lo, n_sel, c->opt.hpc, (uint8_t*)nullptr);
-	HAO_CHECK_LAUNCH();
-	HIP_TRY(hipStreamSynchronize(c->stream));
-	return HAO_OK;
 }
 
 static int hao_prior_hom(const hao_ctx *c)
@@ -302,7 +278,7 @@
 {
 	const uint64_t n = c->n_reads; const int k = c->opt.k;
 	c->has_ft = false; c->h_ft_keys.clear(); c->h_ft_vals.clear();
-	std::vector<uint32_t> slist;
+	const SketchPlan &PL = c->plan; const std::vector<uint32_t> &slist = PL.nlist;
 	DevBuf<uint64_t> slots, chunks, kmer_off, kh_chunk_off, kh, kh2;
 	uint64_t n_slots = 0, n_chunks = 0, n_real = 0;
 	DevBuf<uint64_t> ukeys; DevBuf<uint32_t> ucnt; uint64_t n_unique = 0, *sorted = nullptr;
@@ -320,14 +296,14 @@
 			HIP_TRY(c->d_cursor.reserve(4)); HIP_TRY(hipMemsetAsync(c->d_cursor.p + 2, 0, 8, c->stream));
 			const uint32_t ns = (uint32_t)(s1 - s0);
 			hipLaunchKernelGGL(kmer_hash_scalar_kernel, dim3((ns + 63) / 64), dim3(64), 0, c->stream, c->d_packed.p, c->d_pk_off.p, c->d_len.p,
-							   c->d_nsite_off.p, c->d_nsite.p, c->d_scalar_list.p + (s0 - slist.begin()), ns, kmer_off.p, (uint64_t)0, k, c->opt.hpc, out - slot_base, c->d_cursor.p + 2);
+							   c->d_nsite_off.p, c->d_nsite.p, PL.d_n_list.p + (s0 - slist.begin()), ns, kmer_off.p, (uint64_t)0, k, c->opt.hpc, out - slot_base, c->d_cursor.p + 2);
 			HAO_CHECK_LAUNCH();
 			if (scalar_real) { HIP_TRY(hipMemcpyAsync(scalar_real, c->d_cursor.p + 2, 8, hipMemcpyDeviceToHost, c->stream)); HIP_TRY(hipStreamSynchronize(c->stream)); }
 		}
 		if (n_ch) {
 			hao_kh_args a_;
-			a_.packed = c->d_packed.p; a_.pk_off = c->d_pk_off.p; a_.len = c->d_len.p; a_.tile_off = c->d_tile_off.p; a_.tile_ord = c->d_tile_ord.p; a_.n_runs = c->d_n_runs.p;
-			a_.chunk_off = kh_chunk_off.p; a_.scalar_flag = c->d_scalar_flag.p; a_.kmer_off = kmer_off.p; a_.rid_lo = 0; a_.n_sel = n; a_.k = k; a_.hpc = c->opt.hpc; a_.out = out - slot_base; a_.ch0 = chunk_base;
+			a_.packed = c->d_packed.p; a_.pk_off = c->d_pk_off.p; a_.len = c->d_len.p; a_.tile_off = PL.d_tile_off.p; a_.tile_ord = PL.d_tile_ord.p; a_.n_runs = PL.d_n_runs.p;
+			a_.chunk_off = kh_chunk_off.p; a_.scalar_flag = PL.d_n_flag.p; a_.kmer_off = kmer_off.p; a_.rid_lo = 0; a_.n_sel = n; a_.k = k; a_.hpc = c->opt.hpc; a_.out = out - slot_base; a_.ch0 = chunk_base;
 			hipLaunchKernelGGL(kmer_hash_chunk_kernel, dim3((unsigned)n_ch), dim3(256), hao_kh_smem_bytes(k), c->stream, a_);
 			HAO_CHECK_LAUNCH();
 		}
@@ -336,9 +312,9 @@
 	auto local_index = [&]() -> int {
 		if (n == 0) { hao_set_err(c, "no reads"); return HAO_EINVAL; }
 		if (c->n_bases >= (1ULL << 32) * 16) { hao_set_err(c, "read set too large for one device pass"); return HAO_EUNSUPP; }
-		if (int rc = hao_prepare_runs(c, 0, n, false, slist)) return rc;
+		if (int rc = hao_plan_ensure(c, 0, n, false)) return rc;
 		HIP_TRY(slots.reserve(n + 2)); HIP_TRY(chunks.reserve(n + 2)); HIP_TRY(kmer_off.reserve(n + 2)); HIP_TRY(kh_chunk_off.reserve(n + 2));
-		hipLaunchKernelGGL(hao_kmer_slots_kernel, dim3((unsigned)((n + 256) / 256)), dim3(256), 0, c->stream, c->d_n_runs.p, c->d_scalar_flag.p, c->d_len.p, (uint64_t)0, n, k, slots.p, chunks.p);
+		hipLaunchKernelGGL(hao_kmer_slots_kernel, dim3((unsigned)((n + 256) / 256)), dim3(256), 0, c->stream, PL.d_n_runs.p, PL.d_n_flag.p, c->d_len.p, (uint64_t)0, n, k, slots.p, chunks.p);
 		HAO_CHECK_LAUNCH();
 		if (int rc = hao_excl_scan_u64(c, slots.p, kmer_off.p, n + 1)) return rc;
 		if (int rc = hao_excl_scan_u64(c, chunks.p, kh_chunk_off.p, n + 1)) return rc;
```

New measurement: 180.9 million (median of 3 runs). No clear change (+0.7%).
